# superlinear-ai/raglite

Measured on AMD Instinct MI355X. Metric: queries/sec, MaxSim 32x1M d=1024 exact top-100, higher is better.
Workload: dtype f32 in / f32 scores: candidate chunks found with the fp16 hi halves of corpus and queries (1 x v_mfma_f32_16x16x32_f16 per multiply, f32 accumulate, rigorous error bound), their scores by v_mfma_f32_16x16x4_f32 (exact f32 products); full-precision fallback: 3 x v_mfma_f32_16x16x32_f16 on hi+lo pairs

## Files before the change

include/raglite_hip.h:

```cpp
#ifndef RAGLITE_HIP_H
#define RAGLITE_HIP_H

#include <stddef.h>
#include <stdint.h>

#ifdef __cplusplus
extern "C" {
#endif

typedef enum {
    RL_OK = 0,
    RL_ERR_INVALID = -1,
    RL_ERR_HIP = -2,
    RL_ERR_UNSUPPORTED = -3,
    RL_ERR_NOMEM = -4
} rl_status;

typedef enum { RL_MEM_HOST = 0, RL_MEM_DEVICE = 1 } rl_mem;
#define RL_MEM_FILTERS_DEVICE 2
typedef enum {
    RL_ARITH_AUTO = 0,
    RL_ARITH_FP32_EXACT = 1,
    RL_ARITH_F16_SPLIT = 2,
    RL_ARITH_F16_STORED = 3
} rl_arith;
typedef enum { RL_F32 = 0, RL_F16 = 1 } rl_dtype;
typedef enum { RL_COSINE = 0, RL_DOT = 1, RL_L2 = 2 } rl_metric;
typedef enum { RL_SYNTH_UNIFORM = 0, RL_SYNTH_SMALL_INT = 1 } rl_synth_kind;

typedef struct rl_index rl_index;

int rl_version(void);
const char* rl_last_error(void);
int rl_init(int device);
int rl_device_count(int* count);
int rl_device_info(int device, char* name, int len, int* compute_units, int64_t* total_mem);

int rl_dev_alloc(void** ptr, size_t bytes);
int rl_dev_free(void* ptr);
int rl_memcpy_h2d(void* dst, const void* src, size_t bytes, void* stream);
int rl_memcpy_d2h(void* dst, const void* src, size_t bytes, void* stream);
int rl_memcpy_d2d(void* dst, const void* src, size_t bytes, void* stream);
int rl_stream_sync(void* stream);

int rl_synth_fill(float* dst, int64_t start, int64_t count, uint64_t seed, int kind, void* stream);

int rl_pool_norm(const float* tokens, int64_t n_token_rows, int32_t dim,
                 const int64_t* span_begin, const int64_t* span_end, int64_t n_spans,
                 int32_t normalize, double eps, float* out_f32, uint16_t* out_f16,
                 int mem, void* stream);

int rl_adapter_apply(const float* A, const float* queries, int32_t n_queries, int32_t dim,
                     float* out_f32, uint16_t* out_f16, int mem, void* stream);

int rl_index_create(rl_index** out, const float* embeddings, int64_t n_rows, int32_t dim,
                    const int64_t* chunk_offsets, int64_t n_chunks, int metric, int mem, void* stream);
int rl_index_create_f16(rl_index** out, const uint16_t* embeddings_f16, int64_t n_rows, int32_t dim,
                        const int64_t* chunk_offsets, int64_t n_chunks, int metric, int mem, void* stream);
int rl_index_destroy(rl_index* index);
int rl_index_info(const rl_index* index, int64_t* n_rows, int32_t* dim, int64_t* n_chunks, int* metric);
int rl_index_memory(const rl_index* index, int64_t out[8]);

#define RL_IMAGE_PRESPLIT 1u
#define RL_IMAGE_HI 2u
#define RL_IMAGE_HI_PLANE 4u
int rl_index_prepare(rl_index* index, uint32_t images, uint32_t* built, void* stream);

int rl_index_append(rl_index* index, const float* rows, int64_t n_new_rows, const int64_t* new_chunk_sizes,
                    int64_t n_new_chunks, int mem, void* stream);
int rl_index_delete_chunks(rl_index* index, const int64_t* chunk_ordinals, int64_t n, void* stream);
int rl_index_live(rl_index* index, int64_t* live_rows, int64_t* live_chunks, void* stream);
int rl_index_compact(rl_index* index, int64_t* out_remap, int64_t* new_n_rows, int64_t* new_n_chunks, void* stream);

int rl_index_set_arithmetic(rl_index* index, int mode);
int rl_index_arithmetic(rl_index* index, int* in_effect);

typedef enum {
    RL_OPT_HI_SEARCH = 1, RL_OPT_HI_MAXSIM = 2, RL_OPT_HI_PRODUCTS = 3, RL_OPT_PP_PASS = 4, RL_OPT_FUSED_TOPK = 5, RL_OPT_FUSED_HI = 6,
    RL_OPT_FUSED_PP = 7, RL_OPT_FUSED_TOPK_CAP = 8, RL_OPT_FUSED_TOPK_STRIDE = 9, RL_OPT_GEMM_PASS = 10, RL_OPT_QUERY_PAIRS = 11,
    RL_OPT_PLANES_GEMM = 12, RL_OPT_KEEP_IMAGE = 13, RL_OPT_KEEP_HI = 14, RL_OPT_IMAGE_HEADROOM_MB = 15, RL_OPT_ARITHMETIC = 16,
    RL_OPT_EXACT_KTH_THRESHOLD = 17, RL_OPT_FUSED_TWO_ROUNDS = 18, RL_OPT_KEEP_HI_PLANE = 19, RL_OPT_PAIRS_PACKED = 20,
    RL_OPT_F16_EXACT = 21, RL_OPT_LAZY_IMAGES = 22, RL_OPT_FUSED_PP_SAMPLE = 23,
    RL_OPT_LIST_SELECT = 24, RL_OPT_HI_FEW = 25, RL_OPT_TOPK_BLOCK = 26, RL_OPT_HI_PIVOT = 27, RL_OPT_COUNT_ = 28
} rl_option;
enum { RL_OPT_PP_SCHEDULE = 64, RL_OPT_PP_XCD_PASSES = 65 };
int rl_set_default_option(int key, int64_t value);
int rl_get_default_option(int key, int64_t* value);
int rl_index_set_option(rl_index* index, int key, int64_t value);
int rl_index_get_option(rl_index* index, int key, int64_t* value);

int rl_search_rows(rl_index* index, const float* queries, int32_t n_queries, int32_t k,
                   float* out_scores, int32_t* out_rows, int mem, void* stream);

int rl_rank_cut_begin(rl_index* index, const float* queries, int32_t n_queries, int mem, void* stream);
int rl_rank_cut_level(rl_index* index, int level, int64_t rank_limit, uint32_t* out_hist, int mem, void* stream);
int rl_rank_cut_level_done(rl_index* index, int level, const uint32_t* hist_sum, int mem, void* stream);
int rl_rank_cut_ties(rl_index* index, int64_t rank_limit, uint32_t* out_ties, int mem, void* stream);
int rl_rank_cut_finish(rl_index* index, int64_t rank_limit, const uint32_t* ties_before, const uint32_t* chunk_filter, int32_t k,
                       float* out_scores, int32_t* out_rows, int mem, void* stream);

int rl_search_chunks(rl_index* index, const float* queries, int32_t n_queries, int32_t num_hits,
                     int32_t k, float* out_scores, int32_t* out_chunks, int32_t* out_counts,
                     int mem, void* stream);

int rl_maxsim_topk(rl_index* index, const float* query_vecs, int32_t nq, int32_t k,
                   float* out_scores, int32_t* out_chunks, int mem, void* stream);
int rl_maxsim_scores(rl_index* index, const float* query_vecs, int32_t nq, float* out_scores,
                     int mem, void* stream);
int rl_maxsim_topk_batch(rl_index* index, const float* query_vecs, int32_t n_queries, int32_t nq, int32_t k,
                         float* out_scores, int32_t* out_chunks, int mem, void* stream);
int rl_maxsim_topk_batch_f16(rl_index* index, const uint16_t* query_vecs_f16, int32_t n_queries, int32_t nq, int32_t k,
                             float* out_scores, int32_t* out_chunks, int mem, void* stream);

int rl_maxsim_batch_begin(rl_index* index, const float* query_vecs, int32_t n_queries, int32_t nq, int32_t k, float* out_approx, int mem,
                          void* stream);
int rl_maxsim_batch_finish(rl_index* index, const float* query_vecs, const float* all_approx, int32_t world, int32_t rank, float* out_scores,
                           int32_t* out_chunks, int mem, void* stream);

int rl_maxsim_approx_scores(rl_index* index, const float* query_vecs, int32_t n_queries, int32_t nq, int kernel,
                            float* out_scores, float* out_bound, int mem, void* stream);

int rl_maxsim_rerank(rl_index* index, const float* query_vecs, int32_t n_queries, int32_t nq,
                     const int32_t* candidates, int32_t n_cand, float* out_scores, int mem, void* stream);

int rl_merge_topk(const float* in_scores, const int32_t* in_ids, int32_t n_lists, int32_t n_queries,
                  int32_t k_in, int32_t k, float* out_scores, int32_t* out_ids, int mem, void* stream);

#define RL_COMM_ID_BYTES 128
#define RL_ID_SHARD_MISSING (-2)
typedef struct rl_comm rl_comm;
int rl_comm_unique_id(void* out_id );
int rl_comm_init(rl_comm** out, int rank, int world, const void* unique_id);
int rl_comm_info(const rl_comm* comm, int* rank, int* world);
int rl_comm_destroy(rl_comm* comm);
int rl_allgather_topk(rl_comm* comm, const float* local_scores, const int32_t* local_ids, int32_t n_queries, int32_t k,
                      int32_t id_offset, float* out_scores, int32_t* out_ids, void* stream);
int rl_allgather_merge_topk(rl_comm* comm, const float* local_scores, const int32_t* local_ids, int32_t n_queries,
                            int32_t k_in, int32_t id_offset, int32_t k, float* out_scores, int32_t* out_ids, void* stream);
int rl_allreduce_sum_u32(rl_comm* comm, uint32_t* buf, int64_t count, void* stream);
int rl_allgather_u32(rl_comm* comm, const uint32_t* local, int64_t count, uint32_t* out, void* stream);

int rl_topk(const float* scores, int32_t n_queries, int64_t n, int64_t ld, int32_t k,
            float* out_scores, int32_t* out_ids, int mem, void* stream);

typedef struct rl_keyword_index rl_keyword_index;
int rl_keyword_index_create(rl_keyword_index** out, const int64_t* term_off, int32_t n_terms, const int32_t* post_chunk,
                            const int32_t* post_tf, const int32_t* post_term, int64_t n_postings, const float* idf,
                            const float* nrm, int64_t n_chunks, int mem, void* stream);
int rl_keyword_search(rl_keyword_index* kw, const int64_t* q_off, const int32_t* q_terms, int32_t n_queries, int32_t k,
                      const uint32_t* chunk_filter, float* out_scores, int32_t* out_chunks, int32_t* out_counts, int mem,
                      void* stream);
int rl_keyword_index_info(const rl_keyword_index* kw, int32_t* n_terms, int64_t* n_postings, int64_t* n_chunks);
int rl_keyword_index_destroy(rl_keyword_index* kw);
int rl_keyword_index_read(const rl_keyword_index* kw, int64_t* term_off, int32_t* post_chunk, float* post_impact, int mem,
                          void* stream);

typedef struct rl_keyword_store rl_keyword_store;
int rl_keyword_store_create(rl_keyword_store** out);
int rl_keyword_store_destroy(rl_keyword_store* s);
int rl_keyword_store_info(const rl_keyword_store* s, int64_t* n_chunks, int64_t* n_live, int64_t* n_tokens,
                          int64_t* device_bytes);
int rl_keyword_store_append(rl_keyword_store* s, const int32_t* term_ids, const int64_t* offsets, int64_t n_new_chunks,
                            int mem, void* stream);
int rl_keyword_store_delete(rl_keyword_store* s, const int64_t* chunk_ordinals, int64_t n, void* stream);
int rl_keyword_store_count(rl_keyword_store* s, const int32_t* term_rank, int32_t n_terms, int64_t* out_df,
                           int64_t* out_length, int64_t out_totals[3], int mem, void* stream);
int rl_keyword_store_build(rl_keyword_store* s, const float* idf, const float* nrm, rl_keyword_index** out, int mem,
                           void* stream);

int rl_rrf_fuse(const int32_t* lists, int32_t n_lists, int32_t n_queries, int32_t len, const double* weights, int32_t rrf_k,
                int32_t k, double* out_scores, int32_t* out_ids, int32_t* out_counts, int mem, void* stream);
int rl_hybrid_search(rl_index* index, rl_keyword_index* kw, const float* queries, int32_t n_queries, int32_t num_hits,
                     int32_t n_each, const int64_t* q_off, const int32_t* q_terms, const uint32_t* chunk_filter,
                     int64_t rank_limit, const double* weights, int32_t rrf_k, int32_t k, double* out_scores,
                     int32_t* out_chunks, int32_t* out_counts, int mem, void* stream);

int rl_shard_hybrid_fuse(const int32_t* gathered, int32_t world, int32_t n_queries, int32_t num_hits, int32_t n_each, int32_t n_lists,
                         const double* weights, int32_t rrf_k, int32_t k, double* out_scores, int32_t* out_chunks, int32_t* out_counts,
                         int mem, void* stream);

int rl_search_rows_filtered(rl_index* index, const float* queries, int32_t n_queries, int32_t k,
                            const uint32_t* chunk_filter, float* out_scores, int32_t* out_rows, int mem,
                            void* stream);
int rl_search_chunks_filtered(rl_index* index, const float* queries, int32_t n_queries, int32_t num_hits,
                              int32_t k, const uint32_t* chunk_filter, float* out_scores, int32_t* out_chunks,
                              int32_t* out_counts, int mem, void* stream);
int rl_maxsim_topk_filtered(rl_index* index, const float* query_vecs, int32_t nq, int32_t k,
                            const uint32_t* chunk_filter, float* out_scores, int32_t* out_chunks, int mem,
                            void* stream);

int rl_search_rows_ranked(rl_index* index, const float* queries, int32_t n_queries, int32_t k,
                          const uint32_t* chunk_filter, int64_t rank_limit, float* out_scores, int32_t* out_rows,
                          int mem, void* stream);
int rl_search_chunks_ranked(rl_index* index, const float* queries, int32_t n_queries, int32_t num_hits,
                            int32_t k, const uint32_t* chunk_filter, int64_t rank_limit, float* out_scores,
                            int32_t* out_chunks, int32_t* out_counts, int mem, void* stream);

int rl_search_chunks_per_query(rl_index* index, const float* queries, int32_t n_queries, int32_t num_hits, int32_t k,
                               const uint32_t* chunk_filters, int32_t n_filters, const int32_t* query_filter,
                               const int64_t* rank_limits, float* out_scores, int32_t* out_chunks, int32_t* out_counts,
                               int mem, void* stream);
int rl_keyword_search_per_query(rl_keyword_index* kw, const int64_t* q_off, const int32_t* q_terms, int32_t n_queries,
                                int32_t k, const uint32_t* chunk_filters, int32_t n_filters, const int32_t* query_filter,
                                float* out_scores, int32_t* out_chunks, int32_t* out_counts, int mem, void* stream);
int rl_hybrid_search_per_query(rl_index* index, rl_keyword_index* kw, const float* queries, int32_t n_queries,
                               int32_t num_hits, int32_t n_each, const int64_t* q_off, const int32_t* q_terms,
// ... 62 lines not shown
```

raglite_amd/_abi.py:

```python

from __future__ import annotations

import ctypes as C
import functools
import os
from pathlib import Path

LIB_PATH = Path(os.environ.get("RAGLITE_HIP_LIB") or Path(__file__).resolve().parent / "_lib" / "libraglite_hip.so")

RL_OK, RL_ERR_INVALID, RL_ERR_HIP, RL_ERR_UNSUPPORTED, RL_ERR_NOMEM = 0, -1, -2, -3, -4
MEM_HOST, MEM_DEVICE = 0, 1
MEM_FILTERS_DEVICE = 2
METRICS = {"cosine": 0, "dot": 1, "l2": 2}
SYNTH_KINDS = {"uniform": 0, "small_int": 1}
OPTIONS = {
    "hi_search": 1, "hi_maxsim": 2, "hi_products": 3, "pp_pass": 4, "fused_topk": 5, "fused_hi": 6, "fused_pp": 7, "fused_topk_cap": 8,
    "fused_topk_stride": 9, "gemm_pass": 10, "query_pairs": 11, "planes_gemm": 12, "keep_image": 13, "keep_hi": 14,
    "image_headroom_mb": 15, "arithmetic": 16, "exact_kth_threshold": 17, "fused_two_rounds": 18,
    "keep_hi_plane": 19, "pairs_packed": 20, "f16_exact": 21, "lazy_images": 22, "fused_pp_sample": 23, "list_select": 24, "hi_few": 25, "topk_block": 26, "hi_pivot": 27,
}
SCHEDULE_OPTIONS = {"pp_schedule": 64, "pp_xcd_passes": 65}


def option_key(name: str) -> int:
    return OPTIONS[name] if name in OPTIONS else SCHEDULE_OPTIONS[name]

c_void_p, c_int, c_i32, c_i64, c_u64, c_size_t = C.c_void_p, C.c_int, C.c_int32, C.c_int64, C.c_uint64, C.c_size_t
c_double, c_char_p = C.c_double, C.c_char_p

_SIGNATURES = {
    "rl_version": [],
    "rl_last_error": [],
    "rl_init": [c_int],
    "rl_device_count": [C.POINTER(c_int)],
    "rl_device_info": [c_int, c_char_p, c_int, C.POINTER(c_int), C.POINTER(c_i64)],
    "rl_dev_alloc": [C.POINTER(c_void_p), c_size_t],
    "rl_dev_free": [c_void_p],
    "rl_memcpy_h2d": [c_void_p, c_void_p, c_size_t, c_void_p],
    "rl_memcpy_d2h": [c_void_p, c_void_p, c_size_t, c_void_p],
    "rl_memcpy_d2d": [c_void_p, c_void_p, c_size_t, c_void_p],
    "rl_stream_sync": [c_void_p],
    "rl_synth_fill": [c_void_p, c_i64, c_i64, c_u64, c_int, c_void_p],
    "rl_pool_norm": [c_void_p, c_i64, c_i32, c_void_p, c_void_p, c_i64, c_i32, c_double, c_void_p, c_void_p,
                     c_int, c_void_p],
    "rl_adapter_apply": [c_void_p, c_void_p, c_i32, c_i32, c_void_p, c_void_p, c_int, c_void_p],
    "rl_index_create": [C.POINTER(c_void_p), c_void_p, c_i64, c_i32, c_void_p, c_i64, c_int, c_int, c_void_p],
    "rl_index_destroy": [c_void_p],
    "rl_index_info": [c_void_p, C.POINTER(c_i64), C.POINTER(c_i32), C.POINTER(c_i64), C.POINTER(c_int)],
    "rl_index_memory": [c_void_p, C.POINTER(c_i64)],
    "rl_index_prepare": [c_void_p, C.c_uint32, C.POINTER(C.c_uint32), c_void_p],
    "rl_partition_similarity": [c_void_p, c_i64, c_i32, c_void_p, c_i64, c_void_p, c_void_p, c_int, c_void_p],
    "rl_chunk_best_rows": [c_void_p, c_void_p, c_i32, c_void_p, c_i32, c_void_p, c_int, c_void_p],
    "rl_gather_rows": [c_void_p, c_void_p, c_i64, c_void_p, c_int, c_void_p],
    "rl_index_create_f16": [C.POINTER(c_void_p), c_void_p, c_i64, c_i32, c_void_p, c_i64, c_int, c_int, c_void_p],
    "rl_index_append": [c_void_p, c_void_p, c_i64, c_void_p, c_i64, c_int, c_void_p],
    "rl_index_delete_chunks": [c_void_p, c_void_p, c_i64, c_void_p],
    "rl_index_live": [c_void_p, C.POINTER(c_i64), C.POINTER(c_i64), c_void_p],
    "rl_index_compact": [c_void_p, c_void_p, C.POINTER(c_i64), C.POINTER(c_i64), c_void_p],
    "rl_index_filter_stats": [c_void_p, C.POINTER(c_i64), c_void_p],
    "rl_index_set_arithmetic": [c_void_p, c_int],
    "rl_index_arithmetic": [c_void_p, C.POINTER(c_int)],
    "rl_set_default_option": [c_int, c_i64],
    "rl_get_default_option": [c_int, C.POINTER(c_i64)],
    "rl_index_set_option": [c_void_p, c_int, c_i64],
    "rl_index_get_option": [c_void_p, c_int, C.POINTER(c_i64)],
    "rl_search_rows_filtered": [c_void_p, c_void_p, c_i32, c_i32, c_void_p, c_void_p, c_void_p, c_int, c_void_p],
    "rl_search_chunks_filtered": [c_void_p, c_void_p, c_i32, c_i32, c_i32, c_void_p, c_void_p, c_void_p, c_void_p,
                                  c_int, c_void_p],
    "rl_maxsim_topk_filtered": [c_void_p, c_void_p, c_i32, c_i32, c_void_p, c_void_p, c_void_p, c_int, c_void_p],
    "rl_search_rows_ranked": [c_void_p, c_void_p, c_i32, c_i32, c_void_p, c_i64, c_void_p, c_void_p, c_int, c_void_p],
    "rl_search_chunks_ranked": [c_void_p, c_void_p, c_i32, c_i32, c_i32, c_void_p, c_i64, c_void_p, c_void_p, c_void_p,
                                c_int, c_void_p],
    "rl_search_rows": [c_void_p, c_void_p, c_i32, c_i32, c_void_p, c_void_p, c_int, c_void_p],
    "rl_search_chunks": [c_void_p, c_void_p, c_i32, c_i32, c_i32, c_void_p, c_void_p, c_void_p, c_int, c_void_p],
    "rl_maxsim_topk": [c_void_p, c_void_p, c_i32, c_i32, c_void_p, c_void_p, c_int, c_void_p],
    "rl_maxsim_scores": [c_void_p, c_void_p, c_i32, c_void_p, c_int, c_void_p],
    "rl_maxsim_topk_batch": [c_void_p, c_void_p, c_i32, c_i32, c_i32, c_void_p, c_void_p, c_int, c_void_p],
    "rl_maxsim_topk_batch_f16": [c_void_p, c_void_p, c_i32, c_i32, c_i32, c_void_p, c_void_p, c_int, c_void_p],
    "rl_maxsim_approx_scores": [c_void_p, c_void_p, c_i32, c_i32, c_int, c_void_p, c_void_p, c_int, c_void_p],
    "rl_maxsim_batch_begin": [c_void_p, c_void_p, c_i32, c_i32, c_i32, c_void_p, c_int, c_void_p],
    "rl_maxsim_batch_finish": [c_void_p, c_void_p, c_void_p, c_i32, c_i32, c_void_p, c_void_p, c_int, c_void_p],
    "rl_maxsim_rerank": [c_void_p, c_void_p, c_i32, c_i32, c_void_p, c_i32, c_void_p, c_int, c_void_p],
    "rl_merge_topk": [c_void_p, c_void_p, c_i32, c_i32, c_i32, c_i32, c_void_p, c_void_p, c_int, c_void_p],
    "rl_topk": [c_void_p, c_i32, c_i64, c_i64, c_i32, c_void_p, c_void_p, c_int, c_void_p],
    "rl_time_kernel": [c_void_p, c_int, c_void_p, c_i32, c_i32, C.POINTER(C.c_float), c_void_p],
    "rl_comm_unique_id": [c_void_p],
    "rl_comm_init": [C.POINTER(c_void_p), c_int, c_int, c_void_p],
    "rl_comm_info": [c_void_p, C.POINTER(c_int), C.POINTER(c_int)],
    "rl_comm_destroy": [c_void_p],
    "rl_allgather_topk": [c_void_p, c_void_p, c_void_p, c_i32, c_i32, c_i32, c_void_p, c_void_p, c_void_p],
    "rl_allgather_merge_topk": [c_void_p, c_void_p, c_void_p, c_i32, c_i32, c_i32, c_i32, c_void_p, c_void_p, c_void_p],
    "rl_allreduce_sum_u32": [c_void_p, c_void_p, c_i64, c_void_p],
    "rl_allgather_u32": [c_void_p, c_void_p, c_i64, c_void_p, c_void_p],
    "rl_rank_cut_begin": [c_void_p, c_void_p, c_i32, c_int, c_void_p],
    "rl_rank_cut_level": [c_void_p, c_int, c_i64, c_void_p, c_int, c_void_p],
    "rl_rank_cut_level_done": [c_void_p, c_int, c_void_p, c_int, c_void_p],
    "rl_rank_cut_ties": [c_void_p, c_i64, c_void_p, c_int, c_void_p],
    "rl_rank_cut_finish": [c_void_p, c_i64, c_void_p, c_void_p, c_i32, c_void_p, c_void_p, c_int, c_void_p],
    "rl_keyword_index_create": [C.POINTER(c_void_p), c_void_p, c_i32, c_void_p, c_void_p, c_void_p, c_i64, c_void_p, c_void_p, c_i64,
                                c_int, c_void_p],
    "rl_keyword_search": [c_void_p, c_void_p, c_void_p, c_i32, c_i32, c_void_p, c_void_p, c_void_p, c_void_p, c_int, c_void_p],
    "rl_keyword_index_info": [c_void_p, C.POINTER(c_i32), C.POINTER(c_i64), C.POINTER(c_i64)],
    "rl_keyword_index_destroy": [c_void_p],
    "rl_keyword_index_read": [c_void_p, c_void_p, c_void_p, c_void_p, c_int, c_void_p],
    "rl_keyword_store_create": [C.POINTER(c_void_p)],
    "rl_keyword_store_destroy": [c_void_p],
    "rl_keyword_store_info": [c_void_p, C.POINTER(c_i64), C.POINTER(c_i64), C.POINTER(c_i64), C.POINTER(c_i64)],
    "rl_keyword_store_append": [c_void_p, c_void_p, c_void_p, c_i64, c_int, c_void_p],
    "rl_keyword_store_delete": [c_void_p, c_void_p, c_i64, c_void_p],
    "rl_keyword_store_count": [c_void_p, c_void_p, c_i32, c_void_p, c_void_p, c_void_p, c_int, c_void_p],
    "rl_keyword_store_build": [c_void_p, c_void_p, c_void_p, C.POINTER(c_void_p), c_int, c_void_p],
    "rl_rrf_fuse": [c_void_p, c_i32, c_i32, c_i32, c_void_p, c_i32, c_i32, c_void_p, c_void_p, c_void_p, c_int, c_void_p],
    "rl_shard_hybrid_fuse": [c_void_p, c_i32, c_i32, c_i32, c_i32, c_i32, c_void_p, c_i32, c_i32, c_void_p, c_void_p, c_void_p, c_int,
                             c_void_p],
    "rl_hybrid_search": [c_void_p, c_void_p, c_void_p, c_i32, c_i32, c_i32, c_void_p, c_void_p, c_void_p, c_i64, c_void_p, c_i32, c_i32,
                         c_void_p, c_void_p, c_void_p, c_int, c_void_p],
    "rl_search_chunks_per_query": [c_void_p, c_void_p, c_i32, c_i32, c_i32, c_void_p, c_i32, c_void_p, c_void_p, c_void_p, c_void_p,
                                   c_void_p, c_int, c_void_p],
    "rl_keyword_search_per_query": [c_void_p, c_void_p, c_void_p, c_i32, c_i32, c_void_p, c_i32, c_void_p, c_void_p, c_void_p, c_void_p,
                                    c_int, c_void_p],
    "rl_hybrid_search_per_query": [c_void_p, c_void_p, c_void_p, c_i32, c_i32, c_i32, c_void_p, c_void_p, c_void_p, c_i32, c_void_p,
                                   c_void_p, c_void_p, c_i32, c_i32, c_void_p, c_void_p, c_void_p, c_int, c_void_p],
    "rl_rerank_order": [c_void_p, c_void_p, c_i32, c_i32, c_i32, c_void_p, c_void_p, c_void_p, c_void_p, c_int, c_void_p],
    "rl_search_rerank_per_query": [c_void_p, c_void_p, c_void_p, c_i32, c_i32, c_i32, c_void_p, c_void_p, c_void_p, c_i32, c_void_p,
                                   c_void_p, c_void_p, c_i32, c_i32, c_void_p, c_i32, c_i32, c_void_p, c_void_p, c_void_p, c_int,
                                   c_void_p],
    "rl_span_table_create": [C.POINTER(c_void_p), c_void_p, c_void_p, c_i64],
    "rl_span_table_info": [c_void_p, C.POINTER(c_i64), C.POINTER(c_i64), C.POINTER(c_i64)],
    "rl_span_table_destroy": [c_void_p],
    "rl_chunk_spans": [c_void_p, c_void_p, c_i32, c_i32, c_void_p, c_i32, c_void_p, c_void_p, c_void_p, c_void_p, c_void_p, c_int, c_void_p],
    "rl_search_rerank_spans_per_query": [c_void_p, c_void_p, c_void_p, c_i32, c_i32, c_i32, c_void_p, c_void_p, c_void_p, c_i32, c_void_p,
                                         c_void_p, c_void_p, c_i32, c_i32, c_void_p, c_i32, c_i32, c_void_p, c_void_p, c_i32, c_void_p,
                                         c_void_p, c_void_p, c_void_p, c_void_p, c_void_p, c_void_p, c_int, c_void_p],
    "rl_metadata_store_create": [C.POINTER(c_void_p), c_void_p, c_void_p, c_i64, c_int, c_void_p],
    "rl_metadata_store_append": [c_void_p, c_void_p, c_void_p, c_i64, c_int, c_void_p],
    "rl_metadata_store_memory": [c_void_p, C.POINTER(c_i64)],
    "rl_metadata_store_destroy": [c_void_p],
    "rl_metadata_filters": [c_void_p, c_void_p, c_void_p, c_void_p, c_i32, C.POINTER(c_void_p), c_void_p, c_void_p, c_int, c_void_p],
    "rl_filter_set_bits": [c_void_p, C.POINTER(c_void_p), C.POINTER(c_i32), C.POINTER(c_i64)],
    "rl_filter_set_read": [c_void_p, c_void_p, c_int, c_void_p],
    "rl_filter_set_destroy": [c_void_p],
}
COMM_ID_BYTES = 128
_RESTYPES = {"rl_last_error": c_char_p}
EXPORTED_SYMBOLS = tuple(_SIGNATURES)


class RagliteHipError(RuntimeError):
    """HIP runtime failure inside libraglite_hip.so."""


class UnsupportedError(ValueError):
    """RL_ERR_UNSUPPORTED: the arguments are valid but this entry point does not cover them (a ValueError, as before; its own type so
    that callers with another path -- `ShardedIndex.maxsim_topk_batch` -- can take it)."""


@functools.lru_cache(maxsize=1)
def lib() -> C.CDLL:
    if not LIB_PATH.exists():
        raise ImportError(
            f"{LIB_PATH} not found: build it with `python -m raglite_amd._build` (needs hipcc; "
            "cross-compiles for gfx950 without a GPU). raglite_amd has no CPU fallback."
        )
    try:
        import torch
# ... 48 lines not shown
```

raglite_amd/_ops.py:

```python

from __future__ import annotations

import ctypes as C
import threading
from typing import Any

import numpy as np

from raglite_amd import _abi
from raglite_amd._abi import MEM_DEVICE, MEM_FILTERS_DEVICE, MEM_HOST, METRICS, SYNTH_KINDS, check, lib

K_MAX = 2048


def _is_torch(x: Any) -> bool:
    return type(x).__module__.split(".")[0] == "torch"


def _torch():
    import torch

    return torch


# ... 861 lines not shown
    def maxsim_topk(self, query_vecs, k: int, chunk_filter=None):
        a = _Args()
        p_q, nq, _ = self._queries(a, query_vecs)
        o_s, p_s = a.out((k,), np.float32)
        o_c, p_c = a.out((k,), np.int32)
        p_f = self._filter(a, chunk_filter)
        self._prep(a)
        check(lib().rl_maxsim_topk_filtered(self._handle, p_q, nq, k, p_f, p_s, p_c, a.mem, a.stream))
        return o_s, o_c

    def maxsim_topk_batch(self, query_batch, k: int):
        a = _Args()
        half = _is_half(query_batch)
        p_q = a.inp(query_batch, np.float16 if half else np.float32)
        qv = a.keep[-1]
        if qv.ndim != 3 or int(qv.shape[2]) != self.dim:
            raise ValueError("query_batch must be (n_queries, nq, dim)")
        n_queries, nq = int(qv.shape[0]), int(qv.shape[1])
        o_s, p_s = a.out((n_queries, k), np.float32)
        o_c, p_c = a.out((n_queries, k), np.int32)
        self._prep(a)
        fn = lib().rl_maxsim_topk_batch_f16 if half else lib().rl_maxsim_topk_batch
        check(fn(self._handle, p_q, n_queries, nq, k, p_s, p_c, a.mem, a.stream))
        return o_s, o_c

    def maxsim_approx_scores(self, query_batch, kernel: int = 0):
        a = _Args()
        p_q = a.inp(query_batch, np.float32)
        qv = a.keep[-1]
        if qv.ndim != 3 or int(qv.shape[2]) != self.dim:
            raise ValueError("query_batch must be (n_queries, nq, dim)")
        n_queries, nq = int(qv.shape[0]), int(qv.shape[1])
        o_s, p_s = a.out((n_queries, self.n_chunks), np.float32)
        o_b, p_b = a.out((n_queries,), np.float32)
        self._prep(a)
        check(lib().rl_maxsim_approx_scores(self._handle, p_q, n_queries, nq, int(kernel), p_s, p_b, a.mem, a.stream))
        return o_s, o_b

    def maxsim_batch_begin(self, query_batch, k: int):
        a = _Args()
        p_q = a.inp(query_batch, np.float32)
        qv = a.keep[-1]
        if qv.ndim != 3 or int(qv.shape[2]) != self.dim:
            raise ValueError("query_batch must be (n_queries, nq, dim)")
        n_queries, nq = int(qv.shape[0]), int(qv.shape[1])
        o, p_o = a.out((n_queries, int(k) + 1), np.float32)
        self._prep(a)
        check(lib().rl_maxsim_batch_begin(self._handle, p_q, n_queries, nq, int(k), p_o, a.mem, a.stream))
        return o

    def maxsim_batch_finish(self, query_batch, all_approx, rank: int, k: int):
        a = _Args()
        p_q = a.inp(query_batch, np.float32)
        qv = a.keep[-1]
        n_queries = int(qv.shape[0])
        p_a = a.inp(all_approx, np.float32)
        av = a.keep[-1]
        if av.ndim != 3 or int(av.shape[1]) != n_queries or int(av.shape[2]) != int(k) + 1:
            raise ValueError("all_approx must be (world, n_queries, k + 1)")
        world = int(av.shape[0])
        o_s, p_s = a.out((n_queries, int(k)), np.float32)
        o_c, p_c = a.out((n_queries, int(k)), np.int32)
        self._prep(a)
        check(lib().rl_maxsim_batch_finish(self._handle, p_q, p_a, world, int(rank), p_s, p_c, a.mem, a.stream))
        return o_s, o_c

    def maxsim_rerank(self, query_vecs, candidates):
        a = _Args()
        p_q = a.inp(query_vecs, np.float32)
        qv = a.keep[-1]
        if qv.ndim != 3 or int(qv.shape[2]) != self.dim:
            raise ValueError("query_vecs must be (n_queries, nq, dim)")
        p_c = a.inp(candidates, np.int32)
        cv = a.keep[-1]
        n_queries, nq = int(qv.shape[0]), int(qv.shape[1])
        if cv.ndim != 2 or int(cv.shape[0]) != n_queries:
            raise ValueError("candidates must be (n_queries, n_cand)")
        n_cand = int(cv.shape[1])
        o_s, p_s = a.out((n_queries, n_cand), np.float32)
        self._prep(a)
        check(lib().rl_maxsim_rerank(self._handle, p_q, n_queries, nq, p_c, n_cand, p_s, a.mem, a.stream))
        return o_s

    def chunk_best_rows(self, queries, candidates):
        a = _Args()
        p_q, B, single = self._queries(a, queries)
        c2 = candidates.reshape(1, -1) if candidates.ndim == 1 else candidates
        p_c = a.inp(c2, np.int32)
        if int(a.keep[-1].shape[0]) != B:
            raise ValueError("candidates must have one row per query")
        n_cand = int(a.keep[-1].shape[1])
        o_r, p_r = a.out((B, n_cand), np.int32)
        self._prep(a)
        check(lib().rl_chunk_best_rows(self._handle, p_q, B, p_c, n_cand, p_r, a.mem, a.stream))
        return o_r[0] if single else o_r

    def gather_rows(self, rows):
        a = _Args()
        p_r = a.inp(rows, np.int32)
        n = int(a.keep[0].shape[0])
        o, p_o = a.out((n, self.dim), np.float32)
        self._prep(a)
        check(lib().rl_gather_rows(self._handle, p_r, n, p_o, a.mem, a.stream))
        return o

    def time_kernel(self, kind: int, query_vecs_cuda, iters: int) -> float:
        a = _Args()
        p_q, nq, _ = self._queries(a, query_vecs_cuda)
        if a.mem != MEM_DEVICE:
            raise ValueError("time_kernel needs CUDA tensors")
        ms = C.c_float(0.0)
        self._prep(a)
        check(lib().rl_time_kernel(self._handle, kind, p_q, nq, iters, C.byref(ms), a.stream))
        return float(ms.value)


class KeywordIndex:

    def __init__(self, postings) -> None:
        p = postings
        arrs = [np.ascontiguousarray(p.term_off, dtype=np.int64), np.ascontiguousarray(p.post_chunk, dtype=np.int32),
                np.ascontiguousarray(p.post_tf, dtype=np.int32), np.ascontiguousarray(p.post_term, dtype=np.int32),
                np.ascontiguousarray(p.idf, dtype=np.float32), np.ascontiguousarray(p.nrm, dtype=np.float32)]
        term_off, post_chunk, post_tf, post_term, idf, nrm = arrs
        self.n_terms, self.n_postings, self.n_chunks = int(term_off.size - 1), int(post_chunk.size), int(nrm.size)
        _ensure_init(_current_device())
        handle = C.c_void_p()
        check(lib().rl_keyword_index_create(C.byref(handle), term_off.ctypes.data, self.n_terms, post_chunk.ctypes.data,
                                            post_tf.ctypes.data, post_term.ctypes.data, self.n_postings, idf.ctypes.data,
                                            nrm.ctypes.data, self.n_chunks, MEM_HOST, None))
        self._handle = handle

    @classmethod
    def _from_handle(cls, handle) -> "KeywordIndex":
        self = cls.__new__(cls)
        n_terms, n_postings, n_chunks = C.c_int32(0), C.c_int64(0), C.c_int64(0)
        self._handle = handle
        check(lib().rl_keyword_index_info(handle, C.byref(n_terms), C.byref(n_postings), C.byref(n_chunks)))
        self.n_terms, self.n_postings, self.n_chunks = n_terms.value, n_postings.value, n_chunks.value
        return self

    def read(self):
        term_off = np.empty(self.n_terms + 1, np.int64)
        post_chunk = np.empty(self.n_postings, np.int32)
        post_impact = np.empty(self.n_postings, np.float32)
        _ensure_init(_current_device())
        check(lib().rl_keyword_index_read(self._handle, term_off.ctypes.data, post_chunk.ctypes.data, post_impact.ctypes.data, MEM_HOST, None))
        return term_off, post_chunk, post_impact

    def close(self) -> None:
        h, self._handle = getattr(self, "_handle", None), None
        if h:
            lib().rl_keyword_index_destroy(h)

    def __del__(self) -> None:
        try:
            self.close()
        except Exception:
            pass

    def search(self, query_term_ids, k: int, chunk_filter=None, *, query_filters=None):
        q_off, q_terms = _term_csr(query_term_ids)
        B = int(q_off.size - 1)
        scores = np.empty((B, k), np.float32)
        chunks = np.empty((B, k), np.int32)
        counts = np.empty(B, np.int32)
# ... 96 lines not shown
```

raglite_amd/csrc/api.hip:

```cpp
#include <cmath>
#include <cstdlib>
#include <cstring>
#include <limits>
#include <memory>
#include <mutex>
#include <utility>
#include <vector>

#include "common.h"

namespace rl {

static thread_local std::string g_last_error;
void set_error(const std::string& msg) { g_last_error = msg; }
int fail(int code, const std::string& msg) {
    g_last_error = msg;
    return code;
}

namespace {

hipStream_t as_stream(void* s) { return reinterpret_cast<hipStream_t>(s); }

struct BlockCache {
// ... 100 lines not shown
        if (bytes <= cap) return RL_OK;
        release();
        RL_HIP(hipMalloc(&p, bytes));
        cap = bytes;
        return RL_OK;
    }
    int alloc(size_t bytes, const char* who) {
        release();
        RL_TRY(hip_status(hipMalloc(&p, bytes), who));
        cap = bytes;
        return RL_OK;
    }
    void release() {
        if (p) (void)hipFree(p);
        p = nullptr;
        cap = 0;
    }
    template <class T>
    T* as() const { return reinterpret_cast<T*>(p); }
};
template <class T>
struct DevArray : Pool {
    operator T*() const { return as<T>(); }
};

template <class T>
int stage_in(const T* src, size_t count, int mem, hipStream_t s, DevBuf& tmp, const T** out) {
    if (mem == RL_MEM_DEVICE) { *out = src; return RL_OK; }
    RL_TRY(tmp.alloc(count * sizeof(T)));
    if (count) {
        const void* from = src;
        if (void* pin = g_pinned.take(count * sizeof(T))) {
            std::memcpy(pin, src, count * sizeof(T));
            from = pin;
        }
        RL_HIP(hipMemcpyAsync(tmp.p, from, count * sizeof(T), hipMemcpyHostToDevice, s));
    }
    *out = tmp.as<T>();
    return RL_OK;
}
template <class T>
int stage_out_begin(T* dst, size_t count, int mem, DevBuf& tmp, T** out) {
    if (mem == RL_MEM_DEVICE || dst == nullptr) { *out = dst; return RL_OK; }
    RL_TRY(tmp.alloc(count * sizeof(T)));
    *out = tmp.as<T>();
    return RL_OK;
}
template <class T>
int stage_out_end(T* dst, size_t count, int mem, hipStream_t s, const DevBuf& tmp) {
    if (mem == RL_MEM_DEVICE || dst == nullptr || count == 0) return RL_OK;
    if (void* pin = g_pinned.take(count * sizeof(T))) {
        RL_HIP(hipMemcpyAsync(pin, tmp.p, count * sizeof(T), hipMemcpyDeviceToHost, s));
        g_pinned.pending.push_back({&tmp, pin, dst, count * sizeof(T)});
        return RL_OK;
    }
    RL_HIP(hipMemcpyAsync(dst, tmp.p, count * sizeof(T), hipMemcpyDeviceToHost, s));
    return RL_OK;
}
int sync_and_drain(hipStream_t s) {
    RL_HIP(hipStreamSynchronize(s));
    g_pinned.drain();
    return RL_OK;
}
int finish(int mem, hipStream_t s) {
    if (mem == RL_MEM_HOST) return sync_and_drain(s);
    return RL_OK;
}

int filters_mem(int mem) { return (mem & RL_MEM_FILTERS_DEVICE) ? RL_MEM_DEVICE : mem; }
int args_mem(int mem) { return mem & ~RL_MEM_FILTERS_DEVICE; }

int scan_mode(int metric) {
    switch (metric) {
        case RL_COSINE: return SCAN_COSINE;
        case RL_DOT: return SCAN_DOT;
        case RL_L2: return SCAN_L2;
        default: return -1;
    }
}

constexpr size_t SCORE_BATCH_BYTES = size_t(8) << 30;

struct Options {
    int64_t v[RL_OPT_PP_XCD_PASSES + 1];
    Options() {
        for (auto& x : v) x = 0;
        v[RL_OPT_HI_SEARCH] = v[RL_OPT_HI_MAXSIM] = v[RL_OPT_HI_PRODUCTS] = v[RL_OPT_PP_PASS] = v[RL_OPT_FUSED_TOPK] = v[RL_OPT_FUSED_HI] = 1;
        v[RL_OPT_FUSED_PP] = v[RL_OPT_GEMM_PASS] = v[RL_OPT_QUERY_PAIRS] = v[RL_OPT_PLANES_GEMM] = v[RL_OPT_KEEP_IMAGE] = v[RL_OPT_KEEP_HI] = 1;
        v[RL_OPT_EXACT_KTH_THRESHOLD] = v[RL_OPT_FUSED_TWO_ROUNDS] = v[RL_OPT_KEEP_HI_PLANE] = v[RL_OPT_F16_EXACT] = v[RL_OPT_LAZY_IMAGES] = v[RL_OPT_FUSED_PP_SAMPLE] = v[RL_OPT_LIST_SELECT] = v[RL_OPT_HI_FEW] = 1;
        v[RL_OPT_TOPK_BLOCK] = v[RL_OPT_PAIRS_PACKED] = 2;
        v[RL_OPT_HI_PIVOT] = 1;
        v[RL_OPT_PP_SCHEDULE] = 1;
        v[RL_OPT_PP_XCD_PASSES] = 2;
        v[RL_OPT_IMAGE_HEADROOM_MB] = -1;
        v[RL_OPT_ARITHMETIC] = RL_ARITH_AUTO;
    }
    bool on(int key) const { return v[key] != 0; }
};
std::mutex g_default_opts_mu;
Options g_default_opts;
bool option_key_ok(int key) { return (key >= 1 && key < RL_OPT_COUNT_) || key == RL_OPT_PP_SCHEDULE || key == RL_OPT_PP_XCD_PASSES; }
bool option_value_ok(int key, int64_t value) {
    switch (key) {
        case RL_OPT_HI_SEARCH: case RL_OPT_HI_MAXSIM: case RL_OPT_PP_PASS: case RL_OPT_FUSED_TOPK: case RL_OPT_FUSED_HI: case RL_OPT_FUSED_PP:
        case RL_OPT_GEMM_PASS: case RL_OPT_QUERY_PAIRS: case RL_OPT_PLANES_GEMM: case RL_OPT_KEEP_IMAGE: case RL_OPT_KEEP_HI:
        case RL_OPT_EXACT_KTH_THRESHOLD: case RL_OPT_FUSED_TWO_ROUNDS: case RL_OPT_KEEP_HI_PLANE: case RL_OPT_F16_EXACT: case RL_OPT_LAZY_IMAGES: case RL_OPT_FUSED_PP_SAMPLE: case RL_OPT_LIST_SELECT: case RL_OPT_HI_FEW: case RL_OPT_HI_PIVOT:
        case RL_OPT_PP_SCHEDULE:
            return value == 0 || value == 1;
        case RL_OPT_PP_XCD_PASSES: return value == 8 || value == 4 || value == 2 || value == 1;
        case RL_OPT_TOPK_BLOCK: case RL_OPT_PAIRS_PACKED: return value >= 0 && value <= 2;
        case RL_OPT_HI_PRODUCTS: return value == 1 || value == 2;
        case RL_OPT_FUSED_TOPK_CAP: return value >= 0 && value <= MERGE_CAP;
        case RL_OPT_FUSED_TOPK_STRIDE: return value == 0 || (value >= 2 && value <= (int64_t(1) << 20));
        case RL_OPT_IMAGE_HEADROOM_MB: return value >= -1 && value <= (int64_t(1) << 30);
        case RL_OPT_ARITHMETIC: return value == RL_ARITH_AUTO || value == RL_ARITH_FP32_EXACT;
        default: return false;
    }
}

struct Image {
    Pool buf;
    float scale = 0.f;
    int64_t rows = 0;
    void drop() {
        buf.release();
        scale = 0.f;
        rows = 0;
    }
    bool covers(float at, int64_t n_rows) const { return scale > 0.f && scale == at && rows == n_rows && n_rows > 0; }
};
struct NormStats {
    float max_row_norm = 0.f, max_lo_norm = 0.f, max_lo_ratio = 0.f;
    float min_row_norm = std::numeric_limits<float>::infinity();
    float max_row_norm_scale = 0.f;
    int64_t max_row_norm_rows = 0;
    void reset() { *this = NormStats(); }
    bool measured(int64_t n_rows) const { return max_row_norm_rows == n_rows && max_row_norm > 0.f; }
};

}
}

struct rl_index {
    const float* E = nullptr;
    const uint16_t* E16 = nullptr;
    rl::Pool owned_rows;
    bool owns_E() const { return owned_rows.p != nullptr; }
    int64_t n_rows = 0;
    int32_t dim = 0;
    int64_t n_chunks = 0;
    int metric = RL_COSINE;
    bool has_empty_chunk = false;
    rl::DevArray<int64_t> offsets;
    rl::DevArray<int32_t> row_to_chunk;
    rl::DevArray<float> norm;
    rl::DevArray<float> sumsq;
    int n_cu = 256;
    std::mutex mu;
    rl::SelectWorkspace ws;
    rl::Pool scores;
    rl::Pool hits;
    rl::Pool misc;
    int64_t cap_rows = 0;
    int64_t cap_chunks = 0;
    std::vector<int64_t> h_offsets;
    std::vector<uint32_t> h_live;
    rl::DevArray<uint32_t> live_chunk_bits;
    rl::DevArray<uint32_t> live_row_bits;
    int64_t n_dead_chunks = 0, n_dead_rows = 0;
    rl::Pool maskbuf;
    rl::Pool qsplit;
    rl::DevArray<uint32_t> d_range;
    float max_abs = 0.f, min_row_max = std::numeric_limits<float>::infinity();
    bool nonfinite = false;
    int arithmetic = RL_ARITH_AUTO;
    float split_scale = 0.f;
    rl::Image planes;
    rl::Pool ends, qplanes;
    rl::Pool q32;
    rl::Pool cand;
    rl::Pool fused;
    rl::Pool pp_work;
    rl::Pool rankbuf;
    rl::Pool hybrid;
    rl::Pool rerank;
    rl::Image hiplane;
    rl::Pool hibuf;
    rl::Image hi_image;
    rl::NormStats norm_stats;
    rl::DevArray<uint32_t> d_norms;
// ... 1651 lines not shown
    }
    RL_TRY(maxsim_scores_device(idx, d_q, nq, idx->scores.as<float>(), s));
    const bool masked = d_f || idx->live_chunk_bits;
    RL_TRY(mask_chunk_scores(idx, idx->scores.as<float>(), 1, idx->n_chunks, d_f, s));
    RL_TRY(launch_topk(idx->scores.as<float>(), 1, idx->n_chunks, idx->n_chunks, k, idx->ws, d_s, d_c, s));
    if (masked) RL_TRY(launch_fix_masked(d_s, d_c, k, s));
    RL_TRY(stage_out_end(out_scores, (size_t)k, mem, s, t_s));
    RL_TRY(stage_out_end(out_chunks, (size_t)k, mem, s, t_c));
    return finish(mem, s);
}

int rl_maxsim_topk(rl_index* idx, const float* query_vecs, int32_t nq, int32_t k, float* out_scores,
                   int32_t* out_chunks, int mem, void* stream) {
    return rl_maxsim_topk_filtered(idx, query_vecs, nq, k, nullptr, out_scores, out_chunks, mem, stream);
}

namespace {
struct HiBatch {
    float* ts; int32_t* ti; float* thr; uint32_t* cnt; uint32_t* flag; int32_t* ci; float* es;
    float* m; float* es_top;
    int32_t cap; bool one_product; float m_abs; const float* q_unscale;
    uint64_t* bmax = nullptr;
    const float* qsum = nullptr;
    bool m_ready = true;
    bool exact_kth;
    const uint32_t* filter = nullptr;
};
void hi_batch_layout(rl_index* idx, int32_t n, int32_t k, HiBatch& hb) {
    hb.cap = 2048;
    hb.ts = idx->hibuf.as<float>();
    hb.ti = reinterpret_cast<int32_t*>(hb.ts + (size_t)n * k);
    hb.thr = reinterpret_cast<float*>(hb.ti + (size_t)n * k);
    hb.cnt = reinterpret_cast<uint32_t*>(hb.thr + n);
    hb.flag = hb.cnt + n;
    hb.ci = reinterpret_cast<int32_t*>(hb.flag + 16);
    hb.es = reinterpret_cast<float*>(hb.ci + (size_t)n * hb.cap);
    hb.m = hb.es + (size_t)n * hb.cap;
    hb.es_top = hb.m + n;
    hb.bmax = reinterpret_cast<uint64_t*>((reinterpret_cast<uintptr_t>(hb.es_top + (size_t)n * k) + 7) & ~uintptr_t(7));
}
size_t hi_batch_words(int32_t n, int32_t k) {
    return (size_t)n * k * 3 + (size_t)n * 3 + 16 + (size_t)n * 2048 * 2 + 2 + 2 * pivot_scratch_words(std::min<int32_t>(n, 2));
}
int hi_batch_approx(rl_index* idx, const float* d_q, int32_t nq, int32_t n_queries, int32_t n_gemm, int32_t k, float* sc, int64_t ld, HiBatch& hb,
                    hipStream_t s, bool flag_zeroed = false) {
    hb.one_product = idx->opt.v[RL_OPT_HI_PRODUCTS] == 1;
    hb.exact_kth = idx->opt.on(RL_OPT_EXACT_KTH_THRESHOLD);
    RL_TRY(idx->hibuf.reserve(hi_batch_words(n_gemm, k) * 4));
    hi_batch_layout(idx, n_gemm, k, hb);
    const int32_t cap = hb.cap;
    hb.m_abs = idx->norm_stats.max_lo_norm + sum_eps(idx->dim) * idx->norm_stats.max_row_norm;
    hb.q_unscale = reinterpret_cast<const float*>(idx->qplanes.as<char>() + (size_t)n_queries * idx->dim * 128);
    hb.qsum = hb.q_unscale + 2 * (size_t)n_queries;
    if (!flag_zeroed) RL_HIP(hipMemsetAsync(hb.flag, 0, 16 * sizeof(uint32_t), s));
    (void)cap;
    const bool pp = hb.one_product && idx->dim >= 256 && idx->opt.on(RL_OPT_PP_PASS);
    if (pp)
        RL_TRY(launch_maxsim_pp(approx_image(idx), idx->n_rows, idx->dim, idx->qplanes.p, n_queries, 0, n_gemm, nq, idx->row_to_chunk,
                                idx->offsets, idx->ends.as<uint32_t>(), sc, ld, idx->n_cu, s, approx_scale(idx), nullptr,
                                (int)idx->opt.v[RL_OPT_PP_SCHEDULE], (int)idx->opt.v[RL_OPT_PP_XCD_PASSES]));
    for (int32_t b = 0; !pp && b < n_gemm; b += GEMM_PASS_QUERIES) {
        const int32_t n_q = std::min<int32_t>(GEMM_PASS_QUERIES, n_gemm - b);
        RL_TRY(launch_maxsim_gemm(approx_image(idx), idx->n_rows, idx->dim, idx->qplanes.p, n_queries, b, n_q, nq, idx->row_to_chunk,
                                  idx->offsets, idx->ends.as<uint32_t>(), sc + (int64_t)b * ld, ld, idx->n_cu, s, approx_scale(idx), true,
                                  nullptr, hb.one_product));
    }
    RL_TRY(mask_chunk_scores(idx, sc, n_gemm, ld, hb.filter, s));
    int st_pv = RL_ERR_UNSUPPORTED;
    if (n_gemm < 16 && idx->n_chunks > (int64_t)262144 && idx->opt.on(RL_OPT_HI_PIVOT))
        st_pv = launch_topk_pivot(sc, n_gemm, idx->n_chunks, ld, k, idx->ws, hb.ts, hb.ti, s);
    if (st_pv != RL_OK && st_pv != RL_ERR_UNSUPPORTED) return st_pv;
    if (st_pv == RL_ERR_UNSUPPORTED) RL_TRY(launch_topk(sc, n_gemm, idx->n_chunks, ld, k, idx->ws, hb.ts, hb.ti, s));
    return RL_OK;
}
int hi_batch_fallback(rl_index* idx, const float* d_q, int32_t nq, int32_t n_queries, int32_t n_gemm, int32_t k, float* sc, int64_t ld,
                      const HiBatch& hb, float* d_s, int32_t* d_c, hipStream_t s, bool rows_only = false);
int hi_batch_rescore(rl_index* idx, const float* d_q, int32_t nq, int32_t n_queries, int32_t n_gemm, int32_t k, float* sc, int64_t ld,
                     const HiBatch& hb, float* d_s, int32_t* d_c, hipStream_t s, bool rows_only = false) {
    const size_t q_elems = (size_t)nq * idx->dim;
    const float* rows = idx->E16 ? reinterpret_cast<const float*>(idx->E16) : idx->E;
    const bool rows16 = idx->E16 != nullptr;
    idx->filt = {RL_FILTER_MAXSIM_BATCH, n_gemm, hb.cap, hb.cnt, hb.flag};
    const int packed = (int)idx->opt.v[RL_OPT_PAIRS_PACKED];
    const bool m_from_qsum = !hb.m_ready && hb.qsum != nullptr;
    if (!hb.m_ready && !(hb.exact_kth && k <= hb.cap && hb.qsum)) return fail(RL_ERR_INVALID, "MaxSim batch: no bound for the candidate threshold");
    if (hb.exact_kth && k <= hb.cap) {
        RL_TRY(launch_maxsim_pairs(rows, idx->dim, d_q, nq, (int64_t)q_elems, idx->offsets, hb.ti, k, n_gemm, hb.es_top, s, rows16, 0, 0, packed));
        if (m_from_qsum)
            RL_TRY(launch_exact_threshold(hb.es_top, hb.ti, n_gemm, k, hb.m, hb.cap, hb.thr, hb.cnt, hb.ci, hb.es, hb.flag, s, hb.qsum, hb.m_abs,
                                          idx->norm_stats.max_row_norm + idx->norm_stats.max_lo_norm, hb.one_product, hb.ts));
        else
            RL_TRY(launch_exact_threshold(hb.es_top, hb.ti, n_gemm, k, hb.m, hb.cap, hb.thr, hb.cnt, hb.ci, hb.es, hb.flag, s, nullptr, 0.f, 0.f, false, hb.ts));
        RL_TRY(launch_collect_above(sc, n_gemm, idx->n_chunks, ld, hb.thr, nullptr, hb.cap, hb.ci, nullptr, hb.cnt, hb.flag, s, hb.ts, hb.ti, k));
        if (hb.cap > k)
            RL_TRY(launch_maxsim_pairs(rows, idx->dim, d_q, nq, (int64_t)q_elems, idx->offsets, hb.ci, hb.cap - k, n_gemm, hb.es, s, rows16, hb.cap, k, packed));
    } else {
        RL_HIP(hipMemsetAsync(hb.ci, 0xff, (size_t)n_gemm * hb.cap * sizeof(int32_t), s));
        RL_TRY(launch_collect_above(sc, n_gemm, idx->n_chunks, ld, hb.thr, nullptr, hb.cap, hb.ci, nullptr, hb.cnt, hb.flag, s));
        RL_TRY(launch_maxsim_pairs(rows, idx->dim, d_q, nq, (int64_t)q_elems, idx->offsets, hb.ci, hb.cap, n_gemm, hb.es, s, rows16, 0, 0, packed));
    }
    RL_TRY(launch_merge_topk(hb.es, hb.ci, 1, n_gemm, hb.cap, k, d_s, d_c, s, hb.cnt));
    return hi_batch_fallback(idx, d_q, nq, n_queries, n_gemm, k, sc, ld, hb, d_s, d_c, s, rows_only);
}
int hi_batch_fallback(rl_index* idx, const float* d_q, int32_t nq, int32_t n_queries, int32_t n_gemm, int32_t k, float* sc, int64_t ld,
                      const HiBatch& hb, float* d_s, int32_t* d_c, hipStream_t s, bool rows_only) {
    const size_t q_elems = (size_t)nq * idx->dim;
    if (image_valid(idx) && !rows_only)
        RL_TRY(launch_maxsim_gemm(idx->planes.buf.p, idx->n_rows, idx->dim, idx->qplanes.p, n_queries, 0, n_gemm, nq, idx->row_to_chunk, idx->offsets,
                                  idx->ends.as<uint32_t>(), sc, ld, idx->n_cu, s, image_scale(idx), idx->E16 != nullptr, hb.flag, false, true));
    else if (idx->dim > 1024)
        RL_TRY(launch_maxsim_pairs_all_wide(idx->E, idx->dim, d_q, nq, (int64_t)q_elems, idx->offsets, idx->n_chunks, n_gemm, sc, ld, s, hb.flag));
    else
        RL_TRY(launch_maxsim_stream_batch(idx->E, false, idx->n_rows, idx->dim, d_q, nq, (int64_t)q_elems, n_gemm, idx->row_to_chunk, idx->offsets,
                                          idx->n_chunks, sc, ld, std::max(1, idx->n_cu / std::min<int32_t>(8, std::max<int32_t>(1, n_gemm / 4))), s,
                                          idx->split_scale, hb.flag));
    RL_TRY(mask_chunk_scores(idx, sc, n_gemm, ld, hb.filter, s));
    uint32_t* host_word = nullptr;
    if (idx->opt.on(RL_OPT_LAZY_IMAGES) && !image_valid(idx) && !rows_only) {
        if (!idx->h_fell_back) {
            void* word = nullptr;
            if (hipHostMalloc(&word, sizeof(uint32_t), hipHostMallocMapped) == hipSuccess) {
                idx->h_fell_back.reset(static_cast<uint32_t*>(word));
                *idx->h_fell_back = 0u;
                if (hipHostGetDevicePointer(reinterpret_cast<void**>(&idx->d_fell_back), word, 0) != hipSuccess) {
                    idx->d_fell_back = nullptr;
                    (void)hipGetLastError();
                }
            } else (void)hipGetLastError();
        }
        if (idx->h_fell_back) host_word = idx->d_fell_back;
        if (idx->h_fell_back && !host_word) {
            RL_TRY(launch_guarded_select(sc, n_gemm, idx->n_chunks, ld, k, nullptr, nullptr, nullptr, 0, SCAN_RAW_DOT, 1.0f, d_s, d_c, hb.flag, s));
            RL_HIP(hipMemcpyAsync(idx->h_fell_back.get(), hb.flag, sizeof(uint32_t), hipMemcpyDeviceToHost, s));
            return RL_OK;
        }
    }
    RL_TRY(launch_guarded_select(sc, n_gemm, idx->n_chunks, ld, k, nullptr, nullptr, nullptr, 0, SCAN_RAW_DOT, 1.0f, d_s, d_c, hb.flag, s, host_word));
    return RL_OK;
}

int maxsim_few_hi_plane(rl_index* idx, const float* d_q, int32_t nq, int32_t n, int32_t k, float* sc, int64_t ld, float* d_s, int32_t* d_c,
                        hipStream_t s, const uint32_t* d_filter) {
    if (n < 1 || n > 2 || nq < 1 || nq > 32 || k > 512 || !idx->opt.on(RL_OPT_HI_MAXSIM) || !idx->opt.on(RL_OPT_HI_FEW)) return RL_ERR_UNSUPPORTED;
    if (idx->dim > 1024) return RL_ERR_UNSUPPORTED;
    if (idx->E16 || !idx->E || !(idx->split_scale > 0.f) || idx->has_empty_chunk || idx->n_chunks == 0 || idx->n_rows == 0) return RL_ERR_UNSUPPORTED;
    RL_TRY(demand_images(idx, IMG_HI_PLANE, s));
    if (!hi_valid(idx) || !idx->norm_stats.measured(idx->n_rows)) return RL_ERR_UNSUPPORTED;
    if ((reinterpret_cast<uintptr_t>(d_q) & 15) || (reinterpret_cast<uintptr_t>(idx->E) & 15)) return RL_ERR_UNSUPPORTED;
    const int64_t q_elems = (int64_t)nq * idx->dim;
    int st = RL_ERR_UNSUPPORTED;
    if (n == 2 && nq > 16 && idx->opt.on(RL_OPT_QUERY_PAIRS)) {
        RL_TRY(idx->qsplit.reserve(query_split_bytes(idx->dim, 2)));
        st = launch_query_split(d_q, idx->dim, nq, q_elems, 2, idx->qsplit.as<char>(), true, s);
        if (st == RL_OK)
            st = launch_maxsim_stream2(idx->hiplane.buf.p, true, idx->n_rows, idx->dim, idx->qsplit.as<char>(), 2, 0, nq, idx->row_to_chunk, idx->offsets,
                                       idx->n_chunks, sc, ld, idx->n_cu, s, 1.f);
    }
    if (st == RL_ERR_UNSUPPORTED)
        st = launch_maxsim_stream_batch(idx->hiplane.buf.p, true, idx->n_rows, idx->dim, d_q, nq, q_elems, n, idx->row_to_chunk, idx->offsets,
                                        idx->n_chunks, sc, ld, idx->n_cu, s, 0.f, nullptr);
    if (st != RL_OK) return st;
    HiBatch hb;
    hb.one_product = false;
    hb.exact_kth = idx->opt.on(RL_OPT_EXACT_KTH_THRESHOLD);
    RL_TRY(idx->hibuf.reserve(hi_batch_words(n, k) * 4));
    hi_batch_layout(idx, n, k, hb);
    hb.m_abs = idx->norm_stats.max_lo_norm + sum_eps(idx->dim) * idx->norm_stats.max_row_norm;
    hb.q_unscale = nullptr;
    hb.filter = d_filter;
    if (idx->opt.on(RL_OPT_HI_PIVOT) && !idx->live_chunk_bits && !d_filter && k <= 128) {
        HiBound bound;
        bound.m_out = hb.m;
        PivotMaxSim ms;
        ms.nq = nq; ms.q_stride = q_elems; ms.m_abs = hb.m_abs; ms.fill_ids = hb.ci;
        const int st_pv = launch_pivot_route(sc, n, idx->n_chunks, ld, k, nullptr, nullptr, d_q, idx->dim, SCAN_RAW_DOT, 1.0f / idx->split_scale, hb.bmax,
                                             hb.cnt, n + 16, bound, hb.thr, hb.cap, hb.ci, nullptr, hb.cnt, hb.flag, s, nullptr, nullptr, nullptr, &ms);
        if (st_pv == RL_OK) {
            idx->filt = {RL_FILTER_MAXSIM_BATCH, n, hb.cap, hb.cnt, hb.flag};
            RL_TRY(launch_maxsim_pairs(idx->E, idx->dim, d_q, nq, q_elems, idx->offsets, hb.ci, hb.cap, n, hb.es, s, false, 0, 0,
                                       std::min<int>(1, (int)idx->opt.v[RL_OPT_PAIRS_PACKED])));
            RL_TRY(launch_merge_topk(hb.es, hb.ci, 1, n, hb.cap, k, d_s, d_c, s, hb.cnt));
            return hi_batch_fallback(idx, d_q, nq, n, n, k, sc, ld, hb, d_s, d_c, s, true);
// ... 235 lines not shown
    RL_TRY(stage_out_begin(out_scores, (size_t)n_queries * ld, mem, t_o, &d_o));
    if (out_bound) RL_TRY(stage_out_begin(out_bound, (size_t)n_queries, mem, t_b, &d_b));
    RL_TRY(idx->qplanes.reserve(query_planes_bytes(idx->dim, n_queries)));
    RL_TRY(launch_query_planes(d_q, idx->dim, nq, (int64_t)q_elems, n_queries, idx->qplanes.p, s));
    const int32_t per = kernel == 0 ? n_queries : GEMM_PASS_QUERIES;
    for (int32_t b = 0; b < n_queries; b += per) {
        const int32_t n_q = std::min<int32_t>(per, n_queries - b);
        if (kernel == 0)
            RL_TRY(launch_maxsim_pp(approx_image(idx), idx->n_rows, idx->dim, idx->qplanes.p, n_queries, b, n_q, nq, idx->row_to_chunk, idx->offsets,
                                    idx->ends.as<uint32_t>(), d_o + (int64_t)b * ld, ld, idx->n_cu, s, approx_scale(idx), nullptr,
                                    (int)idx->opt.v[RL_OPT_PP_SCHEDULE], (int)idx->opt.v[RL_OPT_PP_XCD_PASSES]));
        else
            RL_TRY(launch_maxsim_gemm(approx_image(idx), idx->n_rows, idx->dim, idx->qplanes.p, n_queries, b, n_q, nq, idx->row_to_chunk, idx->offsets,
                                      idx->ends.as<uint32_t>(), d_o + (int64_t)b * ld, ld, idx->n_cu, s, approx_scale(idx), true, nullptr, true));
    }
    if (d_b) {
        const float m_abs = idx->norm_stats.max_lo_norm + sum_eps(idx->dim) * idx->norm_stats.max_row_norm;
        const float* q_unscale = reinterpret_cast<const float*>(idx->qplanes.as<char>() + (size_t)n_queries * idx->dim * 128);
        RL_TRY(idx->hibuf.reserve((size_t)n_queries * 4 * sizeof(float) + 64));
        float* top = idx->hibuf.as<float>();
        float* thr = top + n_queries;
        uint32_t* cnt = reinterpret_cast<uint32_t*>(thr + n_queries);
        uint32_t* flag = cnt + n_queries;
        RL_HIP(hipMemsetAsync(top, 0, (size_t)n_queries * sizeof(float), s));
        RL_HIP(hipMemsetAsync(flag, 0, 16 * sizeof(uint32_t), s));
        RL_TRY(launch_maxsim_threshold(top, n_queries, 1, d_q, nq, idx->dim, (int64_t)q_elems, 1.0f, m_abs, thr, cnt, flag, s, q_unscale,
                                       idx->norm_stats.max_row_norm + idx->norm_stats.max_lo_norm));
        RL_TRY(launch_scale_f32(thr, d_b, -0.5f, n_queries, s));
        idx->filt = {};
    }
    RL_TRY(stage_out_end(out_scores, (size_t)n_queries * ld, mem, s, t_o));
    if (out_bound) RL_TRY(stage_out_end(out_bound, (size_t)n_queries, mem, s, t_b));
    return finish(mem, s);
}

}

namespace {
int maxsim_rerank_device(rl_index* idx, const float* d_q, int32_t n_queries, int32_t nq, const int32_t* d_c, int32_t n_cand, float* d_o,
                         hipStream_t s) {
    {
        const int64_t n_items = (int64_t)n_queries * n_cand;
        RL_TRY(idx->cand.reserve((size_t)n_items * sizeof(int32_t)));
        RL_TRY(launch_sanitize_candidates(d_c, n_items, idx->n_chunks, idx->live_chunk_bits, idx->cand.as<int32_t>(), s));
        d_c = idx->cand.as<int32_t>();
    }
    int st = idx->E16 ? launch_maxsim_cand16(idx->E16, idx->dim, d_q, nq, idx->offsets, d_c, n_cand, n_queries, d_o, s)
                      : launch_maxsim_cand(idx->E, idx->dim, d_q, nq, idx->offsets, d_c, n_cand, n_queries, d_o, s, idx->split_scale);
    if (st == RL_ERR_UNSUPPORTED)
        st = launch_maxsim_pairs(idx->E16 ? reinterpret_cast<const float*>(idx->E16) : idx->E, idx->dim, d_q, nq, (int64_t)nq * idx->dim, idx->offsets, d_c,
                                 n_cand, n_queries, d_o, s, idx->E16 != nullptr, 0, 0, (int)idx->opt.v[RL_OPT_PAIRS_PACKED]);
    if (st == RL_ERR_UNSUPPORTED && idx->E16) return fail(st, "rl_maxsim_rerank: unsupported shape for an fp16-stored index");
    if (st == RL_ERR_UNSUPPORTED && !idx->E16)
        st = launch_maxsim_generic(idx->E, idx->dim, d_q, nq, (int64_t)nq * idx->dim, idx->offsets, d_c, n_cand,
                                   n_queries, d_o, s);
    return st;
}
}

extern "C" {

int rl_maxsim_rerank(rl_index* idx, const float* query_vecs, int32_t n_queries, int32_t nq, const int32_t* candidates,
                     int32_t n_cand, float* out_scores, int mem, void* stream) {
    if (!idx) return fail(RL_ERR_INVALID, "rl_maxsim_rerank: null index");
    if (n_queries < 0 || n_cand < 0 || nq < 1) return fail(RL_ERR_INVALID, "rl_maxsim_rerank: bad sizes");
    if (n_queries == 0 || n_cand == 0) return RL_OK;
    if (!query_vecs || !candidates || !out_scores) return fail(RL_ERR_INVALID, "rl_maxsim_rerank: null argument");
    if (idx->E16 && (nq > 32 || idx->dim % 16))
        return fail(RL_ERR_UNSUPPORTED, "rl_maxsim_rerank on an fp16-stored index needs nq <= 32 and dim % 16 == 0");
    if (mem == RL_MEM_HOST) {
        for (int64_t i = 0; i < (int64_t)n_queries * n_cand; ++i)
            if (candidates[i] < -1 || candidates[i] >= idx->n_chunks)
                return fail(RL_ERR_INVALID, "rl_maxsim_rerank: candidate chunk ordinal out of range");
    }
    hipStream_t s = as_stream(stream);
    std::lock_guard<std::mutex> lock(idx->mu);
    RL_TRY(use_scratch(idx, s));
    DevBuf t_q, t_c, t_o;
    const float* d_q; const int32_t* d_c; float* d_o;
    RL_TRY(stage_in(query_vecs, (size_t)n_queries * nq * idx->dim, mem, s, t_q, &d_q));
    RL_TRY(stage_in(candidates, (size_t)n_queries * n_cand, mem, s, t_c, &d_c));
    RL_TRY(stage_out_begin(out_scores, (size_t)n_queries * n_cand, mem, t_o, &d_o));
    RL_TRY(maxsim_rerank_device(idx, d_q, n_queries, nq, d_c, n_cand, d_o, s));
    RL_TRY(stage_out_end(out_scores, (size_t)n_queries * n_cand, mem, s, t_o));
    return finish(mem, s);
}

int rl_merge_topk(const float* in_scores, const int32_t* in_ids, int32_t n_lists, int32_t n_queries, int32_t k_in,
                  int32_t k, float* out_scores, int32_t* out_ids, int mem, void* stream) {
    if (n_lists < 1 || n_queries < 0 || k_in < 1 || k < 1) return fail(RL_ERR_INVALID, "rl_merge_topk: bad sizes");
    if (k > K_MAX) return fail(RL_ERR_UNSUPPORTED, "rl_merge_topk: k must be <= 2048");
    if (n_queries == 0) return RL_OK;
    if (!in_scores || !in_ids || !out_scores || !out_ids) return fail(RL_ERR_INVALID, "rl_merge_topk: null argument");
    hipStream_t s = as_stream(stream);
    const size_t n_in = (size_t)n_lists * n_queries * k_in, n_out = (size_t)n_queries * k;
    DevBuf t_is, t_ii, t_os, t_oi;
    const float* d_is; const int32_t* d_ii; float* d_os; int32_t* d_oi;
    RL_TRY(stage_in(in_scores, n_in, mem, s, t_is, &d_is));
    RL_TRY(stage_in(in_ids, n_in, mem, s, t_ii, &d_ii));
    RL_TRY(stage_out_begin(out_scores, n_out, mem, t_os, &d_os));
    RL_TRY(stage_out_begin(out_ids, n_out, mem, t_oi, &d_oi));
    RL_TRY(launch_merge_topk(d_is, d_ii, n_lists, n_queries, k_in, k, d_os, d_oi, s));
    RL_TRY(stage_out_end(out_scores, n_out, mem, s, t_os));
    RL_TRY(stage_out_end(out_ids, n_out, mem, s, t_oi));
    return finish(mem, s);
}

int rl_topk(const float* scores, int32_t n_queries, int64_t n, int64_t ld, int32_t k, float* out_scores,
            int32_t* out_ids, int mem, void* stream) {
    if (n_queries < 0 || n < 0 || ld < n || k < 1) return fail(RL_ERR_INVALID, "rl_topk: bad sizes");
    if (k > K_MAX) return fail(RL_ERR_UNSUPPORTED, "rl_topk: k must be <= 2048");
    if (n_queries == 0) return RL_OK;
    if ((n > 0 && !scores) || !out_scores || !out_ids) return fail(RL_ERR_INVALID, "rl_topk: null argument");
    hipStream_t s = as_stream(stream);
    const size_t n_in = (size_t)n_queries * ld, n_out = (size_t)n_queries * k;
    DevBuf t_in, t_os, t_oi;
    const float* d_in; float* d_os; int32_t* d_oi;
    RL_TRY(stage_in(scores, n_in, mem, s, t_in, &d_in));
    RL_TRY(stage_out_begin(out_scores, n_out, mem, t_os, &d_os));
    RL_TRY(stage_out_begin(out_ids, n_out, mem, t_oi, &d_oi));
    SelectWorkspace ws;
    {
        std::lock_guard<std::mutex> lock(g_default_opts_mu);
        ws.block_route = (int)g_default_opts.v[RL_OPT_TOPK_BLOCK];
    }
    int st = launch_topk(d_in, n_queries, n, ld, k, ws, d_os, d_oi, s);
    if (st == RL_OK) st = stage_out_end(out_scores, n_out, mem, s, t_os);
    if (st == RL_OK) st = stage_out_end(out_ids, n_out, mem, s, t_oi);
    const int sy = sync_and_drain(s);
    select_workspace_free(ws);
    return st == RL_OK ? sy : st;
}

int rl_partition_similarity(const float* X, int64_t n, int32_t dim, const int64_t* doc_offsets, int64_t n_docs,
                            const uint8_t* nonoutlying, float* out, int mem, void* stream) {
    if (n < 0 || dim <= 0) return fail(RL_ERR_INVALID, "rl_partition_similarity: bad shape");
    if (n == 0) return RL_OK;
    if (!X || !out) return fail(RL_ERR_INVALID, "rl_partition_similarity: null argument");
    if (dim > 4096) return fail(RL_ERR_UNSUPPORTED, "rl_partition_similarity: dim must be <= 4096");
    if (!doc_offsets) n_docs = 1;
    if (n_docs < 1) return fail(RL_ERR_INVALID, "rl_partition_similarity: need at least one document");
    hipStream_t s = as_stream(stream);
    DevBuf t_x, t_off, t_sel, t_out, t_scr, t_one;
    const float* d_x; const int64_t* d_off; const uint8_t* d_sel = nullptr; float* d_out;
    RL_TRY(stage_in(X, (size_t)n * dim, mem, s, t_x, &d_x));
    if (doc_offsets) {
        RL_TRY(stage_in(doc_offsets, (size_t)n_docs + 1, mem, s, t_off, &d_off));
    } else {
        const int64_t one[2] = {0, n};
        RL_TRY(t_one.alloc(sizeof(one)));
        RL_HIP(hipMemcpyAsync(t_one.p, one, sizeof(one), hipMemcpyHostToDevice, s));
        RL_HIP(hipStreamSynchronize(s));
        d_off = t_one.as<int64_t>();
    }
    if (nonoutlying) RL_TRY(stage_in(nonoutlying, (size_t)n, mem, s, t_sel, &d_sel));
    RL_TRY(stage_out_begin(out, (size_t)n, mem, t_out, &d_out));
    RL_TRY(t_scr.alloc(partition_sim_scratch_bytes(n, n_docs, dim)));
    RL_TRY(launch_partition_similarity(d_x, n, dim, d_off, n_docs, d_sel, d_out, t_scr.p, s));
    RL_TRY(stage_out_end(out, (size_t)n, mem, s, t_out));
    return sync_and_drain(s);
}

int rl_chunk_best_rows(rl_index* idx, const float* queries, int32_t B, const int32_t* candidates, int32_t n_cand,
                       int32_t* out_rows, int mem, void* stream) {
    if (!idx) return fail(RL_ERR_INVALID, "rl_chunk_best_rows: null index");
    if (B < 0 || n_cand < 0) return fail(RL_ERR_INVALID, "rl_chunk_best_rows: bad sizes");
// ... 1293 lines not shown
```

raglite_amd/csrc/common.h:

```cpp
#pragma once
#include <hip/hip_runtime.h>
#include <stdint.h>

#include <algorithm>
#include <cstdlib>
#include <string>

#include "raglite_hip.h"

namespace rl {

void set_error(const std::string& msg);
int fail(int code, const std::string& msg);

#define RL_HIP(expr)                                                                         \
    do {                                                                                     \
        hipError_t _e = (expr);                                                              \
        if (_e != hipSuccess)                                                                \
            return ::rl::fail(_e == hipErrorOutOfMemory ? RL_ERR_NOMEM : RL_ERR_HIP,         \
                              std::string(#expr) + ": " + hipGetErrorString(_e));            \
    } while (0)

#define RL_TRY(expr)              \
    do {                          \
// ... 305 lines not shown
int launch_permute_rows(const int32_t* rows_in, const int32_t* pos, int32_t k, int64_t n_items, int32_t* rows_out,
                        hipStream_t s);
int launch_gather_rows(const void* E, bool f16, int32_t dim, int64_t n_rows, const int32_t* rows, int64_t n, float* out,
                       hipStream_t s, const uint32_t* counts = nullptr, int32_t cap = 0);
int launch_compact_rows(const void* src, int64_t row_bytes, const int64_t* old_row, int64_t n, void* dst, hipStream_t s);

size_t partition_sim_scratch_bytes(int64_t n, int64_t n_docs, int32_t dim);
int launch_partition_similarity(const float* X, int64_t n, int32_t dim, const int64_t* doc_off, int64_t n_docs,
                                const uint8_t* sel, float* out, void* scratch, hipStream_t s);

int launch_row_to_chunk(const int64_t* chunk_offsets, int64_t n_chunks, int64_t n_rows, int32_t* row_to_chunk,
                        hipStream_t s);
int launch_maxsim_stream(const float* D, int64_t n_rows, int32_t dim, const float* Q, int32_t nq,
                         const int32_t* row_to_chunk, const int64_t* chunk_offsets, int64_t n_chunks, int mode,
                         float* out, int64_t ld, int n_cu, hipStream_t s, float split_scale = 0.f,
                         const uint32_t* run_if = nullptr);
struct StreamSecondJob {
    const float* D = nullptr;
    int64_t n_rows = 0;
    float* out = nullptr;
    int64_t ld = 0;
    const uint32_t* run_if = nullptr;
};
int launch_maxsim_stream_two(const float* D, int64_t n_rows, int32_t dim, const float* Q, int32_t nq, const int32_t* row_to_chunk,
                             const int64_t* chunk_offsets, int64_t n_chunks, float* out, int64_t ld, int n_cu, hipStream_t s, float split_scale,
                             const StreamSecondJob& job2);
int launch_maxsim_stream_batch(const void* D, bool f16, int64_t n_rows, int32_t dim, const float* Q, int32_t nq, int64_t q_stride,
                               int32_t n_queries, const int32_t* row_to_chunk, const int64_t* chunk_offsets, int64_t n_chunks, float* out,
                               int64_t out_stride, int n_cu, hipStream_t s, float split_scale, const uint32_t* run_if = nullptr);
size_t query_split_bytes(int32_t dim, int32_t n_queries);
int launch_query_split(const float* Q, int32_t dim, int32_t nq, int64_t q_stride, int32_t n_queries, void* buf, bool f16_corpus,
                       hipStream_t s);
int launch_maxsim_stream2(const void* D, bool f16, int64_t n_rows, int32_t dim, const void* split_buf, int32_t n_queries,
                          int32_t first, int32_t nq, const int32_t* row_to_chunk, const int64_t* chunk_offsets, int64_t n_chunks,
                          float* out, int64_t out_stride, int n_cu, hipStream_t s, float split_scale);
size_t planes_bytes(int64_t rows, int32_t dim, bool half = false);
int launch_presplit_rows(const float* E, int64_t first_row, int64_t n_rows, int32_t dim, float scale, void* planes, hipStream_t s);
int launch_preformat_rows16(const uint16_t* E, int64_t first_row, int64_t n_rows, int32_t dim, void* planes, hipStream_t s);
int launch_presplit_hi_rows(const float* E, int64_t first_row, int64_t n_rows, int32_t dim, float scale, void* planes, hipStream_t s);
size_t chunk_ends_words(int64_t rows);
int launch_chunk_ends(const int32_t* row_to_chunk, int64_t n_rows, uint32_t* ends, hipStream_t s);
size_t query_planes_bytes(int32_t dim, int32_t n_queries);
int launch_query_planes(const float* Q, int32_t dim, int32_t nq, int64_t q_stride, int32_t n_queries, void* buf, hipStream_t s,
                        uint32_t* zero_words = nullptr, int n_zero = 0);
int launch_maxsim_gemm(const void* planes, int64_t n_rows, int32_t dim, const void* qbuf, int32_t n_queries, int32_t first,
                       int32_t n_q, int32_t nq, const int32_t* row_to_chunk, const int64_t* chunk_offsets, const uint32_t* ends_bits,
                       float* out, int64_t out_stride, int n_cu, hipStream_t s, float split_scale, bool half = false,
                       const uint32_t* run_if = nullptr, bool hi_only = false, bool all_passes = false);
constexpr int32_t PP_PASS_QUERIES = 16;
int launch_maxsim_pp(const void* image, int64_t n_rows, int32_t dim, const void* qbuf, int32_t n_queries, int32_t first, int32_t n_q,
                     int32_t nq, const int32_t* row_to_chunk, const int64_t* chunk_offsets, const uint32_t* ends_bits, float* out,
                     int64_t out_stride, int n_cu, hipStream_t s, float split_scale, const uint32_t* run_if, int schedule, int xcd_passes);
constexpr int32_t MFMA_RATE_ITERS = 1000;
int launch_mfma_f16_rate(float* out, int n_cu, int32_t iters, hipStream_t s, double* flops);
size_t score_planes_scratch_floats(int32_t nb, int32_t dim);
int launch_score_planes(const void* planes, int64_t n_rows, int32_t dim, const float* Q, int32_t nb, float* scores, int64_t ld,
                        const float* row_norm, const float* row_sumsq, float* scratch, int mode, int n_cu, hipStream_t s, float split_scale,
                        bool half = false);
struct CandArgs { const float* tau; int32_t tau_stride; float* scores; int32_t* ids; uint32_t* cnt; uint32_t* overflow; int32_t cap; };
int launch_score_planes_queries(const float* Q, int32_t nb, int32_t dim, float* scratch, int mode, hipStream_t s, uint32_t* zero_word = nullptr);
size_t pp_rows_scratch_bytes(int64_t n_rows, int32_t nb, int n_cu, int32_t expected_per_query, int32_t* log_cap_out);
int launch_pp_rows_pass(const void* image, int64_t n_rows, int32_t dim, int32_t nb, float* scratch, const float* row_norm, int mode,
                        const CandArgs* cand, void* work, int32_t log_cap, int n_cu, hipStream_t s, float split_scale, int64_t tile_begin = 0,
                        int64_t tile_count = -1, bool norms_ready = false,
                        bool row_norm_test = false);
int launch_pp_rows_sample(const void* image, int64_t n_rows, int32_t dim, int32_t nb, float* scratch, const float* row_norm, int mode, float* S,
                          int64_t ld_s, int32_t stride, int n_cu, hipStream_t s, float split_scale);
int launch_raise_threshold(float* thr, const float* kth, int32_t nq, int32_t k, const float* window, hipStream_t s);
int launch_score_planes_pass(const void* planes, int64_t n_rows, int32_t dim, int32_t nb, float* scratch, float* scores, int64_t ld,
                             const float* row_norm, const float* row_sumsq, int mode, int32_t tile_stride, const uint32_t* run_if,
                             const CandArgs* cand, int n_cu, hipStream_t s, float split_scale, bool half = false, bool hi_only = false);
int launch_row_range(const float* E, int64_t n_rows, int32_t dim, uint32_t* range, hipStream_t s);
int launch_score_gemm(const float* E, int64_t n_rows, int32_t dim, const float* Q, int32_t nb, float* scores,
                      int64_t ld, const float* row_norm, const float* row_sumsq, float* q_sumsq_scratch, int mode,
                      int n_cu, hipStream_t s, float split_scale = 0.f);
size_t score_gemm_scratch_floats(int32_t nb, int32_t dim, bool split);
int launch_maxsim_stream16(const uint16_t* D, int64_t n_rows, int32_t dim, const float* Q, int32_t nq,
                           const int32_t* row_to_chunk, const int64_t* chunk_offsets, int64_t n_chunks, int mode,
                           float* out, int64_t ld, int n_cu, hipStream_t s);
int launch_maxsim_pairs(const float* D, int32_t dim, const float* Q, int32_t nq, int64_t q_stride, const int64_t* chunk_offsets,
                        const int32_t* candidates, int64_t n_items_per_query, int32_t n_queries, float* out, hipStream_t s,
                        bool rows16 = false,
                        int64_t item_stride = 0, int64_t first_item = 0,
                        int packed = 1);
int launch_maxsim_pairs_all_wide(const float* D, int32_t dim, const float* Q, int32_t nq, int64_t q_stride, const int64_t* offsets, int64_t n_chunks,
                                 int32_t n_queries, float* out, int64_t out_stride, hipStream_t s, const uint32_t* run_if, bool rows16 = false);
int launch_maxsim_generic(const float* D, int32_t dim, const float* Q, int32_t nq, int64_t q_stride_queries,
                          const int64_t* chunk_offsets, const int32_t* candidates, int64_t n_items,
                          int32_t n_queries, float* out, hipStream_t s);
int launch_sanitize_candidates(const int32_t* in, int64_t n, int64_t n_chunks, const uint32_t* live_chunk_bits, int32_t* out,
                               hipStream_t s);
int launch_maxsim_cand(const float* D, int32_t dim, const float* Q, int32_t nq, const int64_t* chunk_offsets,
                       const int32_t* candidates, int32_t n_cand, int32_t n_queries, float* out, hipStream_t s,
                       float split_scale = 0.f);
int launch_maxsim_cand16(const uint16_t* D, int32_t dim, const float* Q, int32_t nq, const int64_t* chunk_offsets,
                         const int32_t* candidates, int32_t n_cand, int32_t n_queries, float* out, hipStream_t s);

}
```

raglite_amd/csrc/maxsim_generic.hip:

```cpp
#include "common.h"

namespace rl {

typedef float f32x4 __attribute__((ext_vector_type(4)));
typedef _Float16 h16x8 __attribute__((ext_vector_type(8)));

constexpr int GEN_NQ_MAX = 1024;
constexpr int PAIRS_MAX_DIM = 4096;

template <int NV, int VEC>
__global__ __launch_bounds__(256) void maxsim_generic_kernel(const float* __restrict__ D, int dim,
                                                              const float* __restrict__ Q, int nq,
                                                              const int64_t* __restrict__ offsets,
                                                              const int32_t* __restrict__ candidates,
                                                              int64_t n_items, float* __restrict__ out) {
    __shared__ float msh[4][GEN_NQ_MAX];
    const int lane = threadIdx.x & 63;
    const int w = threadIdx.x >> 6;
    float* m = msh[w];
    const int64_t wave0 = (int64_t)blockIdx.x * 4 + w;
    const int64_t n_waves = (int64_t)gridDim.x * 4;
    for (int64_t item = wave0; item < n_items; item += n_waves) {
        const int64_t chunk = candidates ? (int64_t)candidates[item] : item;
        const int64_t b = chunk >= 0 ? offsets[chunk] : 0, e = chunk >= 0 ? offsets[chunk + 1] : 0;
        for (int i = lane; i < nq; i += 64) m[i] = -INFINITY;
        for (int64_t r = b; r < e; ++r) {
            float x[NV][VEC];
#pragma unroll
            for (int v = 0; v < NV; ++v) {
                const int c = (v * 64 + lane) * VEC;
#pragma unroll
                for (int j = 0; j < VEC; ++j) x[v][j] = 0.f;
                if (c < dim) {
                    if constexpr (VEC == 4) {
                        const float4 t = *reinterpret_cast<const float4*>(D + r * (int64_t)dim + c);
                        x[v][0] = t.x; x[v][1] = t.y; x[v][2] = t.z; x[v][3] = t.w;
                    } else {
                        x[v][0] = D[r * (int64_t)dim + c];
                    }
                }
            }
            for (int i = 0; i < nq; ++i) {
                float s = 0.f;
#pragma unroll
                for (int v = 0; v < NV; ++v) {
                    const int c = (v * 64 + lane) * VEC;
                    if (c < dim) {
                        if constexpr (VEC == 4) {
                            const float4 t = *reinterpret_cast<const float4*>(Q + (int64_t)i * dim + c);
                            s = fmaf(x[v][0], t.x, s); s = fmaf(x[v][1], t.y, s);
                            s = fmaf(x[v][2], t.z, s); s = fmaf(x[v][3], t.w, s);
                        } else {
                            s = fmaf(x[v][0], Q[(int64_t)i * dim + c], s);
                        }
                    }
                }
                s = wave_sum(s);
                if (lane == 0) m[i] = fmaxf(m[i], s);
            }
        }
        float t = 0.f;
        for (int i = lane; i < nq; i += 64) t += m[i];
        t = wave_sum(t);
        if (lane == 0) out[item] = (e > b) ? t : -INFINITY;
    }
}

template <int NV, int VEC>
static int generic_t(const float* D, int32_t dim, const float* Q, int32_t nq, const int64_t* offsets,
                     const int32_t* cand, int64_t n_items, float* out, hipStream_t s) {
    const int blocks = (int)std::max<int64_t>(1, std::min<int64_t>((n_items + 3) / 4, 256 * 8));
    hipLaunchKernelGGL((maxsim_generic_kernel<NV, VEC>), dim3(blocks), dim3(256), 0, s, D, (int)dim, Q, (int)nq,
                       offsets, cand, n_items, out);
    RL_HIP(hipGetLastError());
    return RL_OK;
}

template <bool FULL, int KB, bool ROW16 = false>
__global__ __launch_bounds__(512) void maxsim_pairs_kernel(const float* __restrict__ D, int dim, const float* __restrict__ Q, int nq,
                                                            int64_t q_stride, const int64_t* __restrict__ offsets,
                                                            const int32_t* __restrict__ candidates, int64_t n_items, int64_t item_stride,
                                                            float* __restrict__ out) {
    extern __shared__ __attribute__((aligned(16))) float qs[];
// ... 31 lines not shown
            for (int j = 0; j < NL; ++j) x[j] = (FULL || t0 + 16 * j < dim) ? *reinterpret_cast<const f32x4*>(a + 16 * j) : (f32x4){0.f, 0.f, 0.f, 0.f};
        }
    };
    auto lane_i64 = [](int64_t v, int k) __attribute__((always_inline)) {
        const uint32_t lo = __builtin_amdgcn_readlane((uint32_t)(uint64_t)v, k), hi = __builtin_amdgcn_readlane((uint32_t)((uint64_t)v >> 32), k);
        return (int64_t)(((uint64_t)hi << 32) | lo);
    };
    f32x4 xc[NL], xn[NL];
    for (int64_t base = (int64_t)blockIdx.x * 8 + w; base < n_items; base += 64 * stride) {
        const int64_t mine = base + (int64_t)lane * stride;
        int64_t vb = 0, ve = 0;
        if (mine < n_items) {
            const int64_t chunk = cb[mine];
            if (chunk >= 0) { vb = offsets[chunk]; ve = offsets[chunk + 1]; }
            if (ve <= vb) ob[mine] = -INFINITY;
        }
        const uint64_t todo = __builtin_amdgcn_ballot_w64(ve > vb);
        if (todo == 0ull) continue;
        int k = __builtin_ctzll(todo);
        int64_t e = lane_i64(ve, k), r0 = lane_i64(vb, k);
        int t0 = 0;
        request(xc, e, r0, 0);
        f32x4 y0 = *reinterpret_cast<const f32x4*>(q0), y1 = *reinterpret_cast<const f32x4*>(q1);
        float best0 = -INFINITY, best1 = -INFINITY;
        f32x4 acc0 = (f32x4){0.f, 0.f, 0.f, 0.f}, acc1 = acc0;
        for (;;) {
            const bool more_k = t0 + KB < dim, more_rows = r0 + 16 < e;
            const uint64_t rest = todo & ~((2ull << k) - 1ull);
            const int nk = rest ? __builtin_ctzll(rest) : k;
            const int64_t ne = lane_i64(ve, nk), nb = lane_i64(vb, nk);
            const int64_t n_e = (more_k || more_rows) ? e : ne;
            const int64_t n_r0 = more_k ? r0 : (more_rows ? r0 + 16 : nb);
            const int n_t0 = more_k ? t0 + KB : 0;
            request(xn, n_e, n_r0, n_t0);
            __builtin_amdgcn_sched_barrier(0);
#pragma unroll
            for (int j = 0; j < NL; ++j) {
                if (!FULL && t0 + 16 * j >= dim) break;
                const int tn = j + 1 < NL ? t0 + 16 * (j + 1) : n_t0;
                const int tr = (FULL || tn < dim) ? tn : 0;
                const f32x4 z0 = *reinterpret_cast<const f32x4*>(q0 + tr);
                const f32x4 z1 = *reinterpret_cast<const f32x4*>(q1 + tr);
                __builtin_amdgcn_sched_barrier(0);
#pragma unroll
                for (int u = 0; u < 4; ++u) {
                    acc0 = __builtin_amdgcn_mfma_f32_16x16x4f32(xc[j][u], y0[u], acc0, 0, 0, 0);
                    acc1 = __builtin_amdgcn_mfma_f32_16x16x4f32(xc[j][u], y1[u], acc1, 0, 0, 0);
                }
                __builtin_amdgcn_sched_barrier(0);
                y0 = z0;
                y1 = z1;
            }
            bool last = false;
            if (!more_k) {
                float v0 = -INFINITY, v1 = -INFINITY;
#pragma unroll
                for (int i = 0; i < 4; ++i)
                    if (r0 + 4 * g + i < e) { v0 = fmaxf(v0, acc0[i]); v1 = fmaxf(v1, acc1[i]); }
                v0 = fmaxf(v0, __shfl_xor(v0, 16)); v0 = fmaxf(v0, __shfl_xor(v0, 32));
                v1 = fmaxf(v1, __shfl_xor(v1, 16)); v1 = fmaxf(v1, __shfl_xor(v1, 32));
                best0 = fmaxf(best0, v0);
                best1 = fmaxf(best1, v1);
                acc0 = acc1 = (f32x4){0.f, 0.f, 0.f, 0.f};
                if (!more_rows) {
                    float s0 = best0, s1 = best1;
#pragma unroll
                    for (int o = 1; o < 16; o <<= 1) { s0 += __shfl_xor(s0, o); s1 += __shfl_xor(s1, o); }
                    if (lane == 0) ob[base + (int64_t)k * stride] = s0 + s1;
                    best0 = best1 = -INFINITY;
                    last = rest == 0ull;
                    k = nk;
                }
            }
            if (last) break;
            e = n_e;
            r0 = n_r0;
            t0 = n_t0;
#pragma unroll
            for (int j = 0; j < NL; ++j) xc[j] = xn[j];
        }
    }
}

template <int KB, bool ROW16, int DBG = 0, int NW = 8>
__global__ __launch_bounds__(NW * 64) void maxsim_pairs_packed_kernel(const float* __restrict__ D, int dim, const float* __restrict__ Q, int nq,
                                                                   int64_t q_stride, const int64_t* __restrict__ offsets,
                                                                   const int32_t* __restrict__ candidates, int64_t n_items, int64_t item_stride,
                                                                   float* __restrict__ out) {
    extern __shared__ __attribute__((aligned(16))) float qs[];
    const int pitch = dim + 8;
    const float* Qb = Q + (int64_t)blockIdx.y * q_stride;
    const int32_t* cb = candidates + (int64_t)blockIdx.y * item_stride;
    float* ob = out + (int64_t)blockIdx.y * item_stride;
    if constexpr ((DBG & 16) != 0) return;
    for (int i = threadIdx.x * 4; i < 32 * dim && !(DBG & 4); i += NW * 64 * 4) {
        const int n = i / dim, c = i - n * dim;
        f32x4 v = (f32x4){0.f, 0.f, 0.f, 0.f};
        if (n < nq) v = *reinterpret_cast<const f32x4*>(Qb + (int64_t)n * dim + c);
        *reinterpret_cast<f32x4*>(qs + n * pitch + c) = v;
    }
    __syncthreads();
    if constexpr ((DBG & 8) != 0) return;
    const int lane = threadIdx.x & 63, w = wave_id();
    const int m = lane & 15, g = lane >> 4;
    const float* q0 = qs + m * pitch + 4 * g;
    const float* q1 = qs + (16 + m) * pitch + 4 * g;
    const int64_t stride = (int64_t)gridDim.x * NW;
    constexpr int NL = KB / 16;
    auto request = [&](f32x4 (&x)[NL], int32_t row, int t0) __attribute__((always_inline)) {
        if constexpr ((DBG & 2) != 0) row = m;
        if constexpr (ROW16) {
            typedef _Float16 h16x4 __attribute__((ext_vector_type(4)));
            const _Float16* a = reinterpret_cast<const _Float16*>(D) + (int64_t)row * dim + 4 * g + t0;
#pragma unroll
            for (int j = 0; j < NL; ++j) {
                const h16x4 h = *reinterpret_cast<const h16x4*>(a + 16 * j);
                x[j] = (f32x4){(float)h[0], (float)h[1], (float)h[2], (float)h[3]};
            }
        } else {
            const float* a = D + (int64_t)row * dim + 4 * g + t0;
#pragma unroll
            for (int j = 0; j < NL; ++j) x[j] = *reinterpret_cast<const f32x4*>(a + 16 * j);
        }
    };
    f32x4 xc[NL], xn[NL];
    for (int64_t base = (int64_t)blockIdx.x * NW + w; base < n_items; base += 64 * stride) {
        const int64_t mine = base + (int64_t)lane * stride;
        int32_t vb = 0, ve = 0;
        if (mine < n_items) {
            const int64_t chunk = cb[mine];
            if (chunk >= 0) { vb = (int32_t)offsets[chunk]; ve = (int32_t)offsets[chunk + 1]; }
            if (ve <= vb) ob[mine] = -INFINITY;
        }
        const uint64_t todo = __builtin_amdgcn_ballot_w64(ve > vb);
        if (todo == 0ull) continue;
        uint32_t t_lo = ve > vb ? (uint32_t)(ve - vb) & 0xffffu : 0u, t_hi = ve > vb ? (uint32_t)(ve - vb) >> 16 : 0u;
#pragma unroll
        for (int o = 32; o > 0; o >>= 1) { t_lo += __shfl_xor(t_lo, o); t_hi += __shfl_xor(t_hi, o); }
        const int64_t R = ((int64_t)__builtin_amdgcn_readfirstlane(t_hi) << 16) + (int64_t)__builtin_amdgcn_readfirstlane(t_lo);
        const int64_t n_tiles = (R + 15) >> 4;
        int cur = __builtin_ctzll(todo);
        uint64_t rest = todo & (todo - 1ull);
        int32_t cur_row = __builtin_amdgcn_readlane(vb, cur), cur_end = __builtin_amdgcn_readlane(ve, cur);
        auto next_tile = [&](int32_t& row, int& cand) __attribute__((always_inline)) -> uint32_t {
            uint32_t ends = 0u;
            row = cur_row;
            cand = cur;
#pragma unroll
            for (int sl = 0; sl < 16; ++sl) {
                if (cur >= 0) {
                    if (m == sl) { row = cur_row; cand = cur; }
                    if (++cur_row == cur_end) {
                        ends |= 1u << sl;
                        if (rest != 0ull) {
                            cur = __builtin_ctzll(rest);
                            rest &= rest - 1ull;
                            cur_row = __builtin_amdgcn_readlane(vb, cur);
                            cur_end = __builtin_amdgcn_readlane(ve, cur);
                        } else {
                            cur = -1;
                        }
                    }
                }
            }
            return ends;
        };
        int32_t row_c, row_n = 0;
        int cand_c, cand_n = 0;
        uint32_t ends_c = next_tile(row_c, cand_c), ends_n = 0u;
        int64_t tile = 0;
        int t0 = 0;
        request(xc, row_c, 0);
        f32x4 y0 = *reinterpret_cast<const f32x4*>(q0), y1 = *reinterpret_cast<const f32x4*>(q1);
        float carry0 = -INFINITY, carry1 = -INFINITY;
        f32x4 acc0 = (f32x4){0.f, 0.f, 0.f, 0.f}, acc1 = acc0;
        for (;;) {
            const bool more_k = t0 + KB < dim, more_tiles = tile + 1 < n_tiles;
            if (!more_k && more_tiles) ends_n = next_tile(row_n, cand_n);
            const int32_t n_row = (more_k || !more_tiles) ? row_c : row_n;
            const int n_t0 = more_k ? t0 + KB : 0;
            request(xn, n_row, n_t0);
            __builtin_amdgcn_sched_barrier(0);
#pragma unroll
            for (int j = 0; j < NL; ++j) {
                const int tn = j + 1 < NL ? t0 + 16 * (j + 1) : n_t0;
                const f32x4 z0 = *reinterpret_cast<const f32x4*>(q0 + tn);
                const f32x4 z1 = *reinterpret_cast<const f32x4*>(q1 + tn);
                __builtin_amdgcn_sched_barrier(0);
                if constexpr ((DBG & 1) != 0) {
                    acc0 += xc[j] * y0;
                    acc1 += xc[j] * y1;
                } else {
#pragma unroll
                    for (int u = 0; u < 4; ++u) {
                        acc0 = __builtin_amdgcn_mfma_f32_16x16x4f32(xc[j][u], y0[u], acc0, 0, 0, 0);
                        acc1 = __builtin_amdgcn_mfma_f32_16x16x4f32(xc[j][u], y1[u], acc1, 0, 0, 0);
                    }
                }
                __builtin_amdgcn_sched_barrier(0);
                y0 = z0;
                y1 = z1;
            }
            if (!more_k) {
                const int n_valid = R - 16 * tile < 16 ? (int)(R - 16 * tile) : 16;
                uint32_t em = ends_c;
                int s_lo = 0;
                while (s_lo < n_valid) {
                    const bool closes = em != 0u;
                    const int e = closes ? __builtin_ctz(em) : 15;
                    float v0 = -INFINITY, v1 = -INFINITY;
#pragma unroll
                    for (int i = 0; i < 4; ++i)
                        if (4 * g + i >= s_lo && 4 * g + i <= e) { v0 = fmaxf(v0, acc0[i]); v1 = fmaxf(v1, acc1[i]); }
                    v0 = fmaxf(v0, __shfl_xor(v0, 16)); v0 = fmaxf(v0, __shfl_xor(v0, 32));
                    v1 = fmaxf(v1, __shfl_xor(v1, 16)); v1 = fmaxf(v1, __shfl_xor(v1, 32));
                    const float best0 = fmaxf(carry0, v0), best1 = fmaxf(carry1, v1);
                    if (closes) {
                        float s0 = best0, s1 = best1;
#pragma unroll
                        for (int o = 1; o < 16; o <<= 1) { s0 += __shfl_xor(s0, o); s1 += __shfl_xor(s1, o); }
                        const int c = __builtin_amdgcn_readlane(cand_c, e);
                        if (lane == 0) ob[base + (int64_t)c * stride] = s0 + s1;
                        carry0 = carry1 = -INFINITY;
                        em &= em - 1u;
                    } else {
                        carry0 = best0;
                        carry1 = best1;
                    }
                    s_lo = e + 1;
                }
                acc0 = acc1 = (f32x4){0.f, 0.f, 0.f, 0.f};
                if (!more_tiles) break;
                ++tile;
                row_c = row_n;
                cand_c = cand_n;
                ends_c = ends_n;
            }
            t0 = n_t0;
#pragma unroll
            for (int j = 0; j < NL; ++j) xc[j] = xn[j];
        }
    }
}

constexpr int PW_KW = 128, PW_T = 8, PW_PITCH = PW_KW + 8;
template <bool ROW16>
__global__ __launch_bounds__(512) void maxsim_pairs_wide_kernel(const float* __restrict__ D, int dim, const float* __restrict__ Q, int nq,
                                                                 int64_t q_stride, const int64_t* __restrict__ offsets,
                                                                 const int32_t* __restrict__ candidates, int64_t n_items, int64_t item_stride,
                                                                 float* __restrict__ out, const uint32_t* __restrict__ run_if) {
    extern __shared__ __attribute__((aligned(16))) float qs[];
    if (run_if && __builtin_amdgcn_readfirstlane((int)*run_if) == 0) return;
    const float* Qb = Q + (int64_t)blockIdx.y * q_stride;
    const int32_t* cb = candidates ? candidates + (int64_t)blockIdx.y * item_stride : nullptr;
    float* ob = out + (int64_t)blockIdx.y * item_stride;
    const int lane = threadIdx.x & 63, w = wave_id();
    const int m = lane & 15, g = lane >> 4;
    float* const qw = qs + w * 32 * PW_PITCH;
    const float* q0 = qw + m * PW_PITCH + 4 * g;
    const float* q1 = qw + (16 + m) * PW_PITCH + 4 * g;
    const int64_t stride = (int64_t)gridDim.x * 8;
    const int nwin = dim / PW_KW;
    constexpr int NL = PW_KW / 16;
    auto request = [&](f32x4 (&x)[NL], int32_t row, int t0) __attribute__((always_inline)) {
        if constexpr (ROW16) {
            typedef _Float16 h16x4 __attribute__((ext_vector_type(4)));
            const _Float16* a = reinterpret_cast<const _Float16*>(D) + (int64_t)row * dim + 4 * g + t0;
#pragma unroll
            for (int j = 0; j < NL; ++j) {
                const h16x4 h = *reinterpret_cast<const h16x4*>(a + 16 * j);
                x[j] = (f32x4){(float)h[0], (float)h[1], (float)h[2], (float)h[3]};
            }
        } else {
            const float* a = D + (int64_t)row * dim + 4 * g + t0;
#pragma unroll
            for (int j = 0; j < NL; ++j) x[j] = *reinterpret_cast<const f32x4*>(a + 16 * j);
        }
    };
    f32x4 xc[NL], xn[NL];
    for (int64_t base = (int64_t)blockIdx.x * 8 + w; base < n_items; base += 64 * stride) {
        const int64_t mine = base + (int64_t)lane * stride;
        int32_t vb = 0, ve = 0;
        if (mine < n_items) {
            const int64_t chunk = cb ? (int64_t)cb[mine] : mine;
            if (chunk >= 0) { vb = (int32_t)offsets[chunk]; ve = (int32_t)offsets[chunk + 1]; }
            if (ve <= vb) ob[mine] = -INFINITY;
        }
        const uint64_t todo = __builtin_amdgcn_ballot_w64(ve > vb);
        if (todo == 0ull) continue;
        uint32_t t_lo = ve > vb ? (uint32_t)(ve - vb) & 0xffffu : 0u, t_hi = ve > vb ? (uint32_t)(ve - vb) >> 16 : 0u;
#pragma unroll
        for (int o = 32; o > 0; o >>= 1) { t_lo += __shfl_xor(t_lo, o); t_hi += __shfl_xor(t_hi, o); }
        const int64_t R = ((int64_t)__builtin_amdgcn_readfirstlane(t_hi) << 16) + (int64_t)__builtin_amdgcn_readfirstlane(t_lo);
        const int64_t n_tiles = (R + 15) >> 4;
        int cur = __builtin_ctzll(todo);
        uint64_t rest = todo & (todo - 1ull);
        int32_t cur_row = __builtin_amdgcn_readlane(vb, cur), cur_end = __builtin_amdgcn_readlane(ve, cur);
        auto next_tile = [&](int32_t& row, int& cand) __attribute__((always_inline)) -> uint32_t {
            uint32_t ends = 0u;
            row = cur_row;
            cand = cur;
#pragma unroll
            for (int sl = 0; sl < 16; ++sl) {
                if (cur >= 0) {
                    if (m == sl) { row = cur_row; cand = cur; }
                    if (++cur_row == cur_end) {
                        ends |= 1u << sl;
                        if (rest != 0ull) {
                            cur = __builtin_ctzll(rest);
                            rest &= rest - 1ull;
                            cur_row = __builtin_amdgcn_readlane(vb, cur);
                            cur_end = __builtin_amdgcn_readlane(ve, cur);
                        } else {
                            cur = -1;
                        }
                    }
                }
            }
            return ends;
        };
        float carry0 = -INFINITY, carry1 = -INFINITY;
        for (int64_t tile0 = 0; tile0 < n_tiles; tile0 += PW_T) {
            const int gt = (int)(n_tiles - tile0 < PW_T ? n_tiles - tile0 : PW_T);
            int32_t row[PW_T];
// ... 6 lines not shown
            }
            f32x4 acc[PW_T][2];
#pragma unroll
            for (int t = 0; t < PW_T; ++t) acc[t][0] = acc[t][1] = (f32x4){0.f, 0.f, 0.f, 0.f};
            request(xc, row[0], 0);
            for (int kw = 0; kw < nwin; ++kw) {
                __builtin_amdgcn_wave_barrier();
#pragma unroll
                for (int j = 0; j < 16; ++j) {
                    const int i = j * 64 + lane, n = i >> 5, c = (i & 31) * 4;
                    f32x4 v = (f32x4){0.f, 0.f, 0.f, 0.f};
                    if (n < nq) v = *reinterpret_cast<const f32x4*>(Qb + (int64_t)n * dim + kw * PW_KW + c);
                    *reinterpret_cast<f32x4*>(qw + n * PW_PITCH + c) = v;
                }
                __builtin_amdgcn_wave_barrier();
#pragma unroll
                for (int t = 0; t < PW_T; ++t) {
                    if (t < gt) {
                        const bool last_t = t + 1 >= gt;
                        const int32_t n_row = (t + 1 < PW_T && !last_t) ? row[t + 1 < PW_T ? t + 1 : 0] : row[0];
                        const int n_t0 = last_t ? (kw + 1 < nwin ? (kw + 1) * PW_KW : 0) : kw * PW_KW;
                        request(xn, n_row, n_t0);
                        f32x4 y0 = *reinterpret_cast<const f32x4*>(q0), y1 = *reinterpret_cast<const f32x4*>(q1);
                        __builtin_amdgcn_sched_barrier(0);
#pragma unroll
                        for (int j = 0; j < NL; ++j) {
                            const int tn = j + 1 < NL ? 16 * (j + 1) : 0;
                            const f32x4 z0 = *reinterpret_cast<const f32x4*>(q0 + tn);
                            const f32x4 z1 = *reinterpret_cast<const f32x4*>(q1 + tn);
                            __builtin_amdgcn_sched_barrier(0);
#pragma unroll
                            for (int u = 0; u < 4; ++u) {
                                acc[t][0] = __builtin_amdgcn_mfma_f32_16x16x4f32(xc[j][u], y0[u], acc[t][0], 0, 0, 0);
                                acc[t][1] = __builtin_amdgcn_mfma_f32_16x16x4f32(xc[j][u], y1[u], acc[t][1], 0, 0, 0);
                            }
                            __builtin_amdgcn_sched_barrier(0);
                            y0 = z0;
                            y1 = z1;
                        }
#pragma unroll
                        for (int j = 0; j < NL; ++j) xc[j] = xn[j];
                    }
                }
            }
#pragma unroll
            for (int t = 0; t < PW_T; ++t) {
                if (t < gt) {
                    const int64_t tile = tile0 + t;
                    const int n_valid = R - 16 * tile < 16 ? (int)(R - 16 * tile) : 16;
                    uint32_t em = ends[t];
                    int s_lo = 0;
                    while (s_lo < n_valid) {
                        const bool closes = em != 0u;
                        const int e = closes ? __builtin_ctz(em) : 15;
                        float v0 = -INFINITY, v1 = -INFINITY;
#pragma unroll
                        for (int i = 0; i < 4; ++i)
                            if (4 * g + i >= s_lo && 4 * g + i <= e) { v0 = fmaxf(v0, acc[t][0][i]); v1 = fmaxf(v1, acc[t][1][i]); }
                        v0 = fmaxf(v0, __shfl_xor(v0, 16)); v0 = fmaxf(v0, __shfl_xor(v0, 32));
                        v1 = fmaxf(v1, __shfl_xor(v1, 16)); v1 = fmaxf(v1, __shfl_xor(v1, 32));
                        const float best0 = fmaxf(carry0, v0), best1 = fmaxf(carry1, v1);
                        if (closes) {
                            float s0 = best0, s1 = best1;
#pragma unroll
                            for (int o = 1; o < 16; o <<= 1) { s0 += __shfl_xor(s0, o); s1 += __shfl_xor(s1, o); }
                            const int c = __builtin_amdgcn_readlane(cand[t], e);
                            if (lane == 0) ob[base + (int64_t)c * stride] = s0 + s1;
                            carry0 = carry1 = -INFINITY;
                            em &= em - 1u;
                        } else {
                            carry0 = best0;
                            carry1 = best1;
                        }
                        s_lo = e + 1;
                    }
                }
            }
        }
    }
}

int launch_maxsim_pairs(const float* D, int32_t dim, const float* Q, int32_t nq, int64_t q_stride, const int64_t* offsets,
                        const int32_t* candidates, int64_t n_items_per_query, int32_t n_queries, float* out, hipStream_t s, bool rows16,
                        int64_t item_stride, int64_t first_item, int packed_mode) {
    bool packed = packed_mode != 0;
    if (n_items_per_query <= 0 || n_queries <= 0) return RL_OK;
    if (item_stride <= 0) item_stride = n_items_per_query;
    if (first_item < 0 || first_item + n_items_per_query > item_stride) return RL_ERR_INVALID;
    if (candidates) candidates += first_item;
    if (out) out += first_item;
    if (nq < 1 || nq > 32 || dim % 16 || dim < 16 || dim > PAIRS_MAX_DIM || !candidates) return RL_ERR_UNSUPPORTED;
    if ((reinterpret_cast<uintptr_t>(D) & (rows16 ? 7 : 15)) || (reinterpret_cast<uintptr_t>(Q) & 15) || (q_stride & 3)) return RL_ERR_UNSUPPORTED;
    if (dim > 1024) {
        if (dim % PW_KW) return RL_ERR_UNSUPPORTED;
        const size_t lds_w = (size_t)8 * 32 * PW_PITCH * sizeof(float);
        static bool wide_attr = false;
        if (!wide_attr) {
            RL_HIP(hipFuncSetAttribute(reinterpret_cast<const void*>(maxsim_pairs_wide_kernel<false>), hipFuncAttributeMaxDynamicSharedMemorySize, 160 * 1024));
            RL_HIP(hipFuncSetAttribute(reinterpret_cast<const void*>(maxsim_pairs_wide_kernel<true>), hipFuncAttributeMaxDynamicSharedMemorySize, 160 * 1024));
            wide_attr = true;
        }
        const int per_q = (int)std::max<int64_t>(1, std::min<int64_t>((n_items_per_query + 7) / 8, std::max<int64_t>(1, 256 / n_queries)));
        if (rows16)
            hipLaunchKernelGGL(maxsim_pairs_wide_kernel<true>, dim3(per_q, n_queries), dim3(512), lds_w, s, D, (int)dim, Q, (int)nq, q_stride, offsets,
                               candidates, n_items_per_query, item_stride, out, (const uint32_t*)nullptr);
        else
            hipLaunchKernelGGL(maxsim_pairs_wide_kernel<false>, dim3(per_q, n_queries), dim3(512), lds_w, s, D, (int)dim, Q, (int)nq, q_stride, offsets,
                               candidates, n_items_per_query, item_stride, out, (const uint32_t*)nullptr);
        RL_HIP(hipGetLastError());
        return RL_OK;
    }
    const size_t lds = (size_t)32 * (dim + 8) * sizeof(float);
    static bool attr_set = false;
    if (!attr_set) {
#define RL_PAIRS_ATTR(...) RL_HIP(hipFuncSetAttribute(reinterpret_cast<const void*>(maxsim_pairs_kernel<__VA_ARGS__>), hipFuncAttributeMaxDynamicSharedMemorySize, 160 * 1024))
#define RL_PACKED_ATTR(...) RL_HIP(hipFuncSetAttribute(reinterpret_cast<const void*>(maxsim_pairs_packed_kernel<__VA_ARGS__>), hipFuncAttributeMaxDynamicSharedMemorySize, 160 * 1024))
        RL_PACKED_ATTR(256, false);
        RL_PACKED_ATTR(128, false);
        RL_PACKED_ATTR(256, true);
        RL_PACKED_ATTR(128, true);
        RL_HIP(hipFuncSetAttribute(reinterpret_cast<const void*>(maxsim_pairs_packed_kernel<128, false, 0, 16>), hipFuncAttributeMaxDynamicSharedMemorySize, 160 * 1024));
#undef RL_PACKED_ATTR
        RL_PAIRS_ATTR(true, 256, false);
        RL_PAIRS_ATTR(true, 128, false);
        RL_PAIRS_ATTR(false, 128, false);
        RL_PAIRS_ATTR(true, 256, true);
        RL_PAIRS_ATTR(true, 128, true);
        RL_PAIRS_ATTR(false, 128, true);
#undef RL_PAIRS_ATTR
        attr_set = true;
    }
    const bool full = dim % 128 == 0;
    packed = packed && full;
    const bool wide = packed && packed_mode == 2 && !rows16;
    const int nw = wide ? 16 : 8;
    int per_query = (int)std::max<int64_t>(1, std::min<int64_t>((n_items_per_query + nw - 1) / nw, std::max<int64_t>(1, (packed ? 256 : 512) / n_queries)));
#ifdef RAGLITE_EXPERIMENTS
    if (const char* e = exp_env("RAGLITE_PAIRS_WG_BUDGET")) {
        const int budget = std::atoi(e);
        if (budget > 0) per_query = (int)std::max<int64_t>(1, std::min<int64_t>((n_items_per_query + 7) / 8, std::max<int64_t>(1, budget / n_queries)));
    }
#endif
#define RL_PAIRS(FULL_, KB_)                                                                                                               \
    do {                                                                                                                                   \
        if (rows16)                                                                                                                        \
            hipLaunchKernelGGL((maxsim_pairs_kernel<FULL_, KB_, true>), dim3(per_query, n_queries), dim3(512), lds, s, D, (int)dim, Q, (int)nq, \
                               q_stride, offsets, candidates, n_items_per_query, item_stride, out);                                        \
        else                                                                                                                               \
            hipLaunchKernelGGL((maxsim_pairs_kernel<FULL_, KB_, false>), dim3(per_query, n_queries), dim3(512), lds, s, D, (int)dim, Q, (int)nq, \
                               q_stride, offsets, candidates, n_items_per_query, item_stride, out);                                        \
    } while (0)
#define RL_PACKED(KB_)                                                                                                                     \
    do {                                                                                                                                   \
        if (rows16)                                                                                                                        \
            hipLaunchKernelGGL((maxsim_pairs_packed_kernel<KB_, true>), dim3(per_query, n_queries), dim3(512), lds, s, D, (int)dim, Q, (int)nq, \
                               q_stride, offsets, candidates, n_items_per_query, item_stride, out);                                        \
        else                                                                                                                               \
            hipLaunchKernelGGL((maxsim_pairs_packed_kernel<KB_, false>), dim3(per_query, n_queries), dim3(512), lds, s, D, (int)dim, Q, (int)nq, \
                               q_stride, offsets, candidates, n_items_per_query, item_stride, out);                                        \
    } while (0)
#ifdef RAGLITE_EXPERIMENTS
    static const int pdbg = exp_env("RAGLITE_PAIRS_DBG") ? std::atoi(exp_env("RAGLITE_PAIRS_DBG")) : 0;
    if (packed && dim % 256 == 0 && !rows16 && pdbg) {
#define RL_PDBG(D_) hipLaunchKernelGGL((maxsim_pairs_packed_kernel<256, false, D_>), dim3(per_query, n_queries), dim3(512), lds, s, D, (int)dim, Q, (int)nq, \
                                       q_stride, offsets, candidates, n_items_per_query, item_stride, out)
        static bool dbg_attr = false;
        if (!dbg_attr) {
            RL_HIP(hipFuncSetAttribute(reinterpret_cast<const void*>(maxsim_pairs_packed_kernel<256, false, 1>), hipFuncAttributeMaxDynamicSharedMemorySize, 160 * 1024));
            RL_HIP(hipFuncSetAttribute(reinterpret_cast<const void*>(maxsim_pairs_packed_kernel<256, false, 2>), hipFuncAttributeMaxDynamicSharedMemorySize, 160 * 1024));
            RL_HIP(hipFuncSetAttribute(reinterpret_cast<const void*>(maxsim_pairs_packed_kernel<256, false, 3>), hipFuncAttributeMaxDynamicSharedMemorySize, 160 * 1024));
            RL_HIP(hipFuncSetAttribute(reinterpret_cast<const void*>(maxsim_pairs_packed_kernel<256, false, 4>), hipFuncAttributeMaxDynamicSharedMemorySize, 160 * 1024));
            RL_HIP(hipFuncSetAttribute(reinterpret_cast<const void*>(maxsim_pairs_packed_kernel<256, false, 7>), hipFuncAttributeMaxDynamicSharedMemorySize, 160 * 1024));
            RL_HIP(hipFuncSetAttribute(reinterpret_cast<const void*>(maxsim_pairs_packed_kernel<256, false, 8>), hipFuncAttributeMaxDynamicSharedMemorySize, 160 * 1024));
            RL_HIP(hipFuncSetAttribute(reinterpret_cast<const void*>(maxsim_pairs_packed_kernel<256, false, 16>), hipFuncAttributeMaxDynamicSharedMemorySize, 160 * 1024));
            dbg_attr = true;
        }
        if (pdbg == 1) RL_PDBG(1); else if (pdbg == 2) RL_PDBG(2); else if (pdbg == 3) RL_PDBG(3); else if (pdbg == 4) RL_PDBG(4); else if (pdbg == 8) RL_PDBG(8);
        else if (pdbg == 16) RL_PDBG(16); else RL_PDBG(7);
#undef RL_PDBG
        RL_HIP(hipGetLastError());
        return RL_OK;
    }
#endif
    if (wide)
        hipLaunchKernelGGL((maxsim_pairs_packed_kernel<128, false, 0, 16>), dim3(per_query, n_queries), dim3(1024), lds, s, D, (int)dim, Q, (int)nq, q_stride,
                           offsets, candidates, n_items_per_query, item_stride, out);
    else if (packed && dim % 256 == 0) RL_PACKED(256);
    else if (packed && dim % 128 == 0) RL_PACKED(128);
    else if (dim % 256 == 0) RL_PAIRS(true, 256);
    else if (dim % 128 == 0) RL_PAIRS(true, 128);
    else RL_PAIRS(false, 128);
#undef RL_PACKED
#undef RL_PAIRS
    RL_HIP(hipGetLastError());
    return RL_OK;
}

int launch_maxsim_pairs_all_wide(const float* D, int32_t dim, const float* Q, int32_t nq, int64_t q_stride, const int64_t* offsets, int64_t n_chunks,
                                 int32_t n_queries, float* out, int64_t out_stride, hipStream_t s, const uint32_t* run_if, bool rows16) {
    if (n_chunks <= 0 || n_queries <= 0) return RL_OK;
    if (nq < 1 || nq > 32 || dim <= 1024 || dim > PAIRS_MAX_DIM || dim % PW_KW) return RL_ERR_UNSUPPORTED;
    if ((reinterpret_cast<uintptr_t>(D) & (rows16 ? 7 : 15)) || (reinterpret_cast<uintptr_t>(Q) & 15) || (q_stride & 3)) return RL_ERR_UNSUPPORTED;
    static bool attr = false;
    if (!attr) {
        RL_HIP(hipFuncSetAttribute(reinterpret_cast<const void*>(maxsim_pairs_wide_kernel<false>), hipFuncAttributeMaxDynamicSharedMemorySize, 160 * 1024));
        RL_HIP(hipFuncSetAttribute(reinterpret_cast<const void*>(maxsim_pairs_wide_kernel<true>), hipFuncAttributeMaxDynamicSharedMemorySize, 160 * 1024));
        attr = true;
    }
    const size_t lds_w = (size_t)8 * 32 * PW_PITCH * sizeof(float);
    const int per_q = (int)std::max<int64_t>(1, std::min<int64_t>((n_chunks + 511) / 512, std::max<int64_t>(1, 1024 / n_queries)));
    if (rows16)
        hipLaunchKernelGGL(maxsim_pairs_wide_kernel<true>, dim3(per_q, n_queries), dim3(512), lds_w, s, D, (int)dim, Q, (int)nq, q_stride, offsets,
                           (const int32_t*)nullptr, n_chunks, out_stride, out, run_if);
    else
    hipLaunchKernelGGL(maxsim_pairs_wide_kernel<false>, dim3(per_q, n_queries), dim3(512), lds_w, s, D, (int)dim, Q, (int)nq, q_stride, offsets,
                       (const int32_t*)nullptr, n_chunks, out_stride, out, run_if);
    RL_HIP(hipGetLastError());
    return RL_OK;
}

int launch_maxsim_generic(const float* D, int32_t dim, const float* Q, int32_t nq, int64_t q_stride,
                          const int64_t* offsets, const int32_t* candidates, int64_t n_items_per_query,
                          int32_t n_queries, float* out, hipStream_t s) {
    if (nq < 1 || nq > GEN_NQ_MAX) return fail(RL_ERR_UNSUPPORTED, "MaxSim: nq must be in [1, 1024]");
    if (n_items_per_query <= 0 || n_queries <= 0) return RL_OK;
    const bool vec4 = (dim % 4 == 0) && ((reinterpret_cast<uintptr_t>(D) & 15) == 0) &&
                      ((reinterpret_cast<uintptr_t>(Q) & 15) == 0) && ((q_stride * 4) % 16 == 0);
    for (int32_t qi = 0; qi < n_queries; ++qi) {
        const float* Qq = Q + (int64_t)qi * q_stride;
        const int32_t* cq = candidates ? candidates + (int64_t)qi * n_items_per_query : nullptr;
        float* oq = out + (int64_t)qi * n_items_per_query;
        int st = RL_ERR_UNSUPPORTED;
        if (vec4) {
            const int nv = (dim + 255) / 256;
            if (nv <= 1) st = generic_t<1, 4>(D, dim, Qq, nq, offsets, cq, n_items_per_query, oq, s);
            else if (nv <= 2) st = generic_t<2, 4>(D, dim, Qq, nq, offsets, cq, n_items_per_query, oq, s);
            else if (nv <= 4) st = generic_t<4, 4>(D, dim, Qq, nq, offsets, cq, n_items_per_query, oq, s);
            else if (nv <= 8) st = generic_t<8, 4>(D, dim, Qq, nq, offsets, cq, n_items_per_query, oq, s);
            else if (nv <= 16) st = generic_t<16, 4>(D, dim, Qq, nq, offsets, cq, n_items_per_query, oq, s);
        } else {
            const int nv = (dim + 63) / 64;
            if (nv <= 2) st = generic_t<2, 1>(D, dim, Qq, nq, offsets, cq, n_items_per_query, oq, s);
            else if (nv <= 8) st = generic_t<8, 1>(D, dim, Qq, nq, offsets, cq, n_items_per_query, oq, s);
            else if (nv <= 32) st = generic_t<32, 1>(D, dim, Qq, nq, offsets, cq, n_items_per_query, oq, s);
        }
        if (st == RL_ERR_UNSUPPORTED) return fail(RL_ERR_UNSUPPORTED, "MaxSim: dim too large for the generic kernel");
        RL_TRY(st);
    }
    return RL_OK;
}

constexpr int CD = 128;
constexpr int CPW = 8;

template <int NQT, bool F16, bool SPLIT = false>
__global__ __launch_bounds__(256) void maxsim_cand_kernel(const float* __restrict__ D, const float* __restrict__ Q,
                                                           int nq, const int64_t* __restrict__ offsets,
                                                           const int32_t* __restrict__ candidates, int n_cand,
                                                           int n_queries, float* __restrict__ out, float e_scale) {
    static_assert(!(F16 && SPLIT), "SPLIT is a way to multiply an fp32-stored corpus");
    const int lane = threadIdx.x & 63;
    const int fj = lane & 15, kq = lane >> 4;
    const int groups = (n_cand + CPW - 1) / CPW;
    const int64_t wave = (int64_t)blockIdx.x * 4 + (threadIdx.x >> 6);
    if (wave >= (int64_t)n_queries * groups) return;
    const int qi = (int)(wave / groups);
    const int c0 = (int)(wave % groups) * CPW;

    constexpr bool H = F16 || SPLIT;
// ... 109 lines not shown
                    for (int h = 0; h < NQT; ++h) acl[h] = __builtin_amdgcn_mfma_f32_16x16x32_f16(el, qhi[h][m], acl[h], 0, 0, 0);
                    if (any_lo) {
#pragma unroll
                        for (int h = 0; h < NQT; ++h) acl[h] = __builtin_amdgcn_mfma_f32_16x16x32_f16(eh, qlo[h][m], acl[h], 0, 0, 0);
                    }
                }
#pragma unroll
                for (int h = 0; h < NQT; ++h) acc[h] = (acc[h] + acl[h]) * q_unscale;
            } else if constexpr (!F16) {
                const float* p = D + row * CD + 4 * kq;
                f32x4 a[8];
#pragma unroll
                for (int mm = 0; mm < 8; ++mm) a[mm] = *reinterpret_cast<const f32x4*>(p + 16 * mm);
#pragma unroll
                for (int mm = 0; mm < 8; ++mm)
#pragma unroll
                    for (int tt = 0; tt < 4; ++tt)
#pragma unroll
                        for (int h = 0; h < NQT; ++h)
                            acc[h] = __builtin_amdgcn_mfma_f32_16x16x4f32(a[mm][tt], qreg[h][4 * mm + tt], acc[h], 0, 0, 0);
            } else {
                const uint16_t* p = reinterpret_cast<const uint16_t*>(D) + row * CD + 8 * kq;
                h16x8 a[4];
#pragma unroll
                for (int mm = 0; mm < 4; ++mm) a[mm] = *reinterpret_cast<const h16x8*>(p + 32 * mm);
#pragma unroll
                for (int mm = 0; mm < 4; ++mm)
#pragma unroll
                    for (int h = 0; h < NQT; ++h)
                        acc[h] = __builtin_amdgcn_mfma_f32_16x16x32_f16(a[mm], qhi[h][mm], acc[h], 0, 0, 0);
                if (any_lo) {
#pragma unroll
                    for (int mm = 0; mm < 4; ++mm)
#pragma unroll
                        for (int h = 0; h < NQT; ++h)
                            acc[h] = __builtin_amdgcn_mfma_f32_16x16x32_f16(a[mm], qlo[h][mm], acc[h], 0, 0, 0);
                }
            }
#pragma unroll
            for (int h = 0; h < NQT; ++h)
#pragma unroll
                for (int r = 0; r < 4; ++r) {
                    const bool valid = (r0 + 4 * kq + r) < e;
                    mx[h][r] = fmaxf(mx[h][r], valid ? acc[h][r] : -INFINITY);
                }
        }
        float s = 0.f;
#pragma unroll
        for (int h = 0; h < NQT; ++h) {
            float v = fmaxf(fmaxf(mx[h][0], mx[h][1]), fmaxf(mx[h][2], mx[h][3]));
            v = fmaxf(v, __shfl_xor(v, 16, 64));
            v = fmaxf(v, __shfl_xor(v, 32, 64));
            s += (16 * h + fj < nq) ? v : 0.f;
        }
        s += __shfl_xor(s, 1, 64);
        s += __shfl_xor(s, 2, 64);
        s += __shfl_xor(s, 4, 64);
        s += __shfl_xor(s, 8, 64);
        if (lane == 0) out[(int64_t)qi * n_cand + ci] = (e > b) ? s : -INFINITY;
    }
}

static int launch_cand_any(const float* D, bool f16, int32_t dim, const float* Q, int32_t nq, const int64_t* offsets,
                           const int32_t* candidates, int32_t n_cand, int32_t n_queries, float* out, hipStream_t s,
                           float split_scale = 0.f) {
    if (dim != CD || nq < 1 || nq > 32) return RL_ERR_UNSUPPORTED;
    if ((reinterpret_cast<uintptr_t>(D) & 15) || (reinterpret_cast<uintptr_t>(Q) & 15)) return RL_ERR_UNSUPPORTED;
    if (n_cand <= 0 || n_queries <= 0) return RL_OK;
    const int64_t waves = (int64_t)n_queries * ((n_cand + CPW - 1) / CPW);
    const int64_t blocks = (waves + 3) / 4;
    if (blocks > 0x7fffffff) return fail(RL_ERR_UNSUPPORTED, "MaxSim rerank: too many (query, candidate) pairs per launch");
#define RL_CAND(NQT, ...) hipLaunchKernelGGL((maxsim_cand_kernel<NQT, __VA_ARGS__>), dim3((unsigned)blocks), dim3(256), 0, s, D, Q, \
                                             (int)nq, offsets, candidates, (int)n_cand, (int)n_queries, out, split_scale)
    if (f16) { if (nq <= 16) RL_CAND(1, true); else RL_CAND(2, true); }
    else if (split_scale > 0.f) { if (nq <= 16) RL_CAND(1, false, true); else RL_CAND(2, false, true); }
    else     { if (nq <= 16) RL_CAND(1, false); else RL_CAND(2, false); }
#undef RL_CAND
    RL_HIP(hipGetLastError());
    return RL_OK;
}

__global__ __launch_bounds__(256) void sanitize_candidates_kernel(const int32_t* __restrict__ in, int64_t n, int64_t n_chunks,
                                                                   const uint32_t* __restrict__ live_chunk_bits,
                                                                   int32_t* __restrict__ out) {
    const int64_t i = (int64_t)blockIdx.x * blockDim.x + threadIdx.x;
    if (i >= n) return;
    const int32_t c = in[i];
    bool ok = c >= 0 && c < n_chunks;
    if (ok && live_chunk_bits) ok = (live_chunk_bits[c >> 5] >> (c & 31)) & 1u;
    out[i] = ok ? c : -1;
}
int launch_sanitize_candidates(const int32_t* in, int64_t n, int64_t n_chunks, const uint32_t* live_chunk_bits, int32_t* out,
                               hipStream_t s) {
    if (n <= 0) return RL_OK;
    hipLaunchKernelGGL(sanitize_candidates_kernel, dim3((unsigned)((n + 255) / 256)), dim3(256), 0, s, in, n, n_chunks, live_chunk_bits, out);
    RL_HIP(hipGetLastError());
    return RL_OK;
}

int launch_maxsim_cand(const float* D, int32_t dim, const float* Q, int32_t nq, const int64_t* offsets,
                       const int32_t* candidates, int32_t n_cand, int32_t n_queries, float* out, hipStream_t s,
                       float split_scale) {
    return launch_cand_any(D, false, dim, Q, nq, offsets, candidates, n_cand, n_queries, out, s, split_scale);
}

int launch_maxsim_cand16(const uint16_t* D, int32_t dim, const float* Q, int32_t nq, const int64_t* offsets,
                         const int32_t* candidates, int32_t n_cand, int32_t n_queries, float* out, hipStream_t s) {
    return launch_cand_any(reinterpret_cast<const float*>(D), true, dim, Q, nq, offsets, candidates, n_cand, n_queries,
                           out, s);
}

}
```

Before: 18260.

## Flatten MaxSim pair rerank into count-aware load-balanced persistent workgroups

```diff
diff --git a/include/raglite_hip.h b/include/raglite_hip.h
--- a/include/raglite_hip.h
+++ b/include/raglite_hip.h
@@ -83,7 +83,7 @@
     RL_OPT_F16_EXACT = 21, RL_OPT_LAZY_IMAGES = 22, RL_OPT_FUSED_PP_SAMPLE = 23,
     RL_OPT_LIST_SELECT = 24, RL_OPT_HI_FEW = 25, RL_OPT_TOPK_BLOCK = 26, RL_OPT_HI_PIVOT = 27, RL_OPT_COUNT_ = 28
 } rl_option;
-enum { RL_OPT_PP_SCHEDULE = 64, RL_OPT_PP_XCD_PASSES = 65 };
+enum { RL_OPT_PP_SCHEDULE = 64, RL_OPT_PP_XCD_PASSES = 65, RL_OPT_PAIRS_FLAT = 66 };
 int rl_set_default_option(int key, int64_t value);
 int rl_get_default_option(int key, int64_t* value);
 int rl_index_set_option(rl_index* index, int key, int64_t value);
@@ -122,6 +122,8 @@
 
 int rl_maxsim_rerank(rl_index* index, const float* query_vecs, int32_t n_queries, int32_t nq,
                      const int32_t* candidates, int32_t n_cand, float* out_scores, int mem, void* stream);
+int rl_maxsim_rerank_counted(rl_index* index, const float* query_vecs, int32_t n_queries, int32_t nq, const int32_t* candidates, int32_t n_cand,
+                             const uint32_t* counts, int32_t n_workgroups, float* out_scores, int mem, void* stream);
 
 int rl_merge_topk(const float* in_scores, const int32_t* in_ids, int32_t n_lists, int32_t n_queries,
                   int32_t k_in, int32_t k, float* out_scores, int32_t* out_ids, int mem, void* stream);
diff --git a/raglite_amd/_abi.py b/raglite_amd/_abi.py
--- a/raglite_amd/_abi.py
+++ b/raglite_amd/_abi.py
@@ -19,7 +19,7 @@
     "image_headroom_mb": 15, "arithmetic": 16, "exact_kth_threshold": 17, "fused_two_rounds": 18,
     "keep_hi_plane": 19, "pairs_packed": 20, "f16_exact": 21, "lazy_images": 22, "fused_pp_sample": 23, "list_select": 24, "hi_few": 25, "topk_block": 26, "hi_pivot": 27,
 }
-SCHEDULE_OPTIONS = {"pp_schedule": 64, "pp_xcd_passes": 65}
+SCHEDULE_OPTIONS = {"pp_schedule": 64, "pp_xcd_passes": 65, "pairs_flat": 66}
 
 
 def option_key(name: str) -> int:
@@ -81,6 +81,7 @@
     "rl_maxsim_batch_begin": [c_void_p, c_void_p, c_i32, c_i32, c_i32, c_void_p, c_int, c_void_p],
     "rl_maxsim_batch_finish": [c_void_p, c_void_p, c_void_p, c_i32, c_i32, c_void_p, c_void_p, c_int, c_void_p],
     "rl_maxsim_rerank": [c_void_p, c_void_p, c_i32, c_i32, c_void_p, c_i32, c_void_p, c_int, c_void_p],
+    "rl_maxsim_rerank_counted": [c_void_p, c_void_p, c_i32, c_i32, c_void_p, c_i32, c_void_p, c_i32, c_void_p, c_int, c_void_p],
     "rl_merge_topk": [c_void_p, c_void_p, c_i32, c_i32, c_i32, c_i32, c_void_p, c_void_p, c_int, c_void_p],
     "rl_topk": [c_void_p, c_i32, c_i64, c_i64, c_i32, c_void_p, c_void_p, c_int, c_void_p],
     "rl_time_kernel": [c_void_p, c_int, c_void_p, c_i32, c_i32, C.POINTER(C.c_float), c_void_p],
diff --git a/raglite_amd/_ops.py b/raglite_amd/_ops.py
--- a/raglite_amd/_ops.py
+++ b/raglite_amd/_ops.py
@@ -967,6 +967,26 @@
         check(lib().rl_maxsim_rerank(self._handle, p_q, n_queries, nq, p_c, n_cand, p_s, a.mem, a.stream))
         return o_s
 
+    def maxsim_rerank_counted(self, query_vecs, candidates, counts, n_workgroups: int = 0):
+        a = _Args()
+        p_q = a.inp(query_vecs, np.float32)
+        qv = a.keep[-1]
+        if qv.ndim != 3 or int(qv.shape[2]) != self.dim:
+            raise ValueError("query_vecs must be (n_queries, nq, dim)")
+        p_c = a.inp(candidates, np.int32)
+        cv = a.keep[-1]
+        n_queries, nq = int(qv.shape[0]), int(qv.shape[1])
+        if cv.ndim != 2 or int(cv.shape[0]) != n_queries:
+            raise ValueError("candidates must be (n_queries, n_cand)")
+        p_n = a.inp(counts, np.int32)
+        if a.keep[-1].ndim != 1 or int(a.keep[-1].shape[0]) != n_queries:
+            raise ValueError("counts must be (n_queries,)")
+        n_cand = int(cv.shape[1])
+        o_s, p_s = a.out((n_queries, n_cand), np.float32)
+        self._prep(a)
+        check(lib().rl_maxsim_rerank_counted(self._handle, p_q, n_queries, nq, p_c, n_cand, p_n, int(n_workgroups), p_s, a.mem, a.stream))
+        return o_s
+
     def chunk_best_rows(self, queries, candidates):
         a = _Args()
         p_q, B, single = self._queries(a, queries)
diff --git a/raglite_amd/csrc/api.hip b/raglite_amd/csrc/api.hip
--- a/raglite_amd/csrc/api.hip
+++ b/raglite_amd/csrc/api.hip
@@ -206,7 +206,7 @@
 constexpr size_t SCORE_BATCH_BYTES = size_t(8) << 30;
 
 struct Options {
-    int64_t v[RL_OPT_PP_XCD_PASSES + 1];
+    int64_t v[RL_OPT_PAIRS_FLAT + 1];
     Options() {
         for (auto& x : v) x = 0;
         v[RL_OPT_HI_SEARCH] = v[RL_OPT_HI_MAXSIM] = v[RL_OPT_HI_PRODUCTS] = v[RL_OPT_PP_PASS] = v[RL_OPT_FUSED_TOPK] = v[RL_OPT_FUSED_HI] = 1;
@@ -216,6 +216,7 @@
         v[RL_OPT_HI_PIVOT] = 1;
         v[RL_OPT_PP_SCHEDULE] = 1;
         v[RL_OPT_PP_XCD_PASSES] = 2;
+        v[RL_OPT_PAIRS_FLAT] = 1;
         v[RL_OPT_IMAGE_HEADROOM_MB] = -1;
         v[RL_OPT_ARITHMETIC] = RL_ARITH_AUTO;
     }
@@ -223,13 +224,13 @@
 };
 std::mutex g_default_opts_mu;
 Options g_default_opts;
-bool option_key_ok(int key) { return (key >= 1 && key < RL_OPT_COUNT_) || key == RL_OPT_PP_SCHEDULE || key == RL_OPT_PP_XCD_PASSES; }
+bool option_key_ok(int key) { return (key >= 1 && key < RL_OPT_COUNT_) || key == RL_OPT_PP_SCHEDULE || key == RL_OPT_PP_XCD_PASSES || key == RL_OPT_PAIRS_FLAT; }
 bool option_value_ok(int key, int64_t value) {
     switch (key) {
         case RL_OPT_HI_SEARCH: case RL_OPT_HI_MAXSIM: case RL_OPT_PP_PASS: case RL_OPT_FUSED_TOPK: case RL_OPT_FUSED_HI: case RL_OPT_FUSED_PP:
         case RL_OPT_GEMM_PASS: case RL_OPT_QUERY_PAIRS: case RL_OPT_PLANES_GEMM: case RL_OPT_KEEP_IMAGE: case RL_OPT_KEEP_HI:
         case RL_OPT_EXACT_KTH_THRESHOLD: case RL_OPT_FUSED_TWO_ROUNDS: case RL_OPT_KEEP_HI_PLANE: case RL_OPT_F16_EXACT: case RL_OPT_LAZY_IMAGES: case RL_OPT_FUSED_PP_SAMPLE: case RL_OPT_LIST_SELECT: case RL_OPT_HI_FEW: case RL_OPT_HI_PIVOT:
-        case RL_OPT_PP_SCHEDULE:
+        case RL_OPT_PP_SCHEDULE: case RL_OPT_PAIRS_FLAT:
             return value == 0 || value == 1;
         case RL_OPT_PP_XCD_PASSES: return value == 8 || value == 4 || value == 2 || value == 1;
         case RL_OPT_TOPK_BLOCK: case RL_OPT_PAIRS_PACKED: return value >= 0 && value <= 2;
@@ -2047,10 +2048,11 @@
     const bool rows16 = idx->E16 != nullptr;
     idx->filt = {RL_FILTER_MAXSIM_BATCH, n_gemm, hb.cap, hb.cnt, hb.flag};
     const int packed = (int)idx->opt.v[RL_OPT_PAIRS_PACKED];
+    const int flat = idx->opt.on(RL_OPT_PAIRS_FLAT) ? idx->n_cu : 0;
     const bool m_from_qsum = !hb.m_ready && hb.qsum != nullptr;
     if (!hb.m_ready && !(hb.exact_kth && k <= hb.cap && hb.qsum)) return fail(RL_ERR_INVALID, "MaxSim batch: no bound for the candidate threshold");
     if (hb.exact_kth && k <= hb.cap) {
-        RL_TRY(launch_maxsim_pairs(rows, idx->dim, d_q, nq, (int64_t)q_elems, idx->offsets, hb.ti, k, n_gemm, hb.es_top, s, rows16, 0, 0, packed));
+        RL_TRY(launch_maxsim_pairs(rows, idx->dim, d_q, nq, (int64_t)q_elems, idx->offsets, hb.ti, k, n_gemm, hb.es_top, s, rows16, 0, 0, packed, nullptr, 0, flat));
         if (m_from_qsum)
             RL_TRY(launch_exact_threshold(hb.es_top, hb.ti, n_gemm, k, hb.m, hb.cap, hb.thr, hb.cnt, hb.ci, hb.es, hb.flag, s, hb.qsum, hb.m_abs,
                                           idx->norm_stats.max_row_norm + idx->norm_stats.max_lo_norm, hb.one_product, hb.ts));
@@ -2058,11 +2060,12 @@
             RL_TRY(launch_exact_threshold(hb.es_top, hb.ti, n_gemm, k, hb.m, hb.cap, hb.thr, hb.cnt, hb.ci, hb.es, hb.flag, s, nullptr, 0.f, 0.f, false, hb.ts));
         RL_TRY(launch_collect_above(sc, n_gemm, idx->n_chunks, ld, hb.thr, nullptr, hb.cap, hb.ci, nullptr, hb.cnt, hb.flag, s, hb.ts, hb.ti, k));
         if (hb.cap > k)
-            RL_TRY(launch_maxsim_pairs(rows, idx->dim, d_q, nq, (int64_t)q_elems, idx->offsets, hb.ci, hb.cap - k, n_gemm, hb.es, s, rows16, hb.cap, k, packed));
+            RL_TRY(launch_maxsim_pairs(rows, idx->dim, d_q, nq, (int64_t)q_elems, idx->offsets, hb.ci, hb.cap - k, n_gemm, hb.es, s, rows16, hb.cap, k, packed,
+                                       hb.cnt, k, flat));
     } else {
         RL_HIP(hipMemsetAsync(hb.ci, 0xff, (size_t)n_gemm * hb.cap * sizeof(int32_t), s));
         RL_TRY(launch_collect_above(sc, n_gemm, idx->n_chunks, ld, hb.thr, nullptr, hb.cap, hb.ci, nullptr, hb.cnt, hb.flag, s));
-        RL_TRY(launch_maxsim_pairs(rows, idx->dim, d_q, nq, (int64_t)q_elems, idx->offsets, hb.ci, hb.cap, n_gemm, hb.es, s, rows16, 0, 0, packed));
+        RL_TRY(launch_maxsim_pairs(rows, idx->dim, d_q, nq, (int64_t)q_elems, idx->offsets, hb.ci, hb.cap, n_gemm, hb.es, s, rows16, 0, 0, packed, hb.cnt, 0, flat));
     }
     RL_TRY(launch_merge_topk(hb.es, hb.ci, 1, n_gemm, hb.cap, k, d_s, d_c, s, hb.cnt));
     return hi_batch_fallback(idx, d_q, nq, n_queries, n_gemm, k, sc, ld, hb, d_s, d_c, s, rows_only);
@@ -2464,6 +2467,34 @@
     RL_TRY(stage_in(candidates, (size_t)n_queries * n_cand, mem, s, t_c, &d_c));
     RL_TRY(stage_out_begin(out_scores, (size_t)n_queries * n_cand, mem, t_o, &d_o));
     RL_TRY(maxsim_rerank_device(idx, d_q, n_queries, nq, d_c, n_cand, d_o, s));
+    RL_TRY(stage_out_end(out_scores, (size_t)n_queries * n_cand, mem, s, t_o));
+    return finish(mem, s);
+}
+
+int rl_maxsim_rerank_counted(rl_index* idx, const float* query_vecs, int32_t n_queries, int32_t nq, const int32_t* candidates, int32_t n_cand,
+                             const uint32_t* counts, int32_t n_workgroups, float* out_scores, int mem, void* stream) {
+    if (!idx) return fail(RL_ERR_INVALID, "rl_maxsim_rerank_counted: null index");
+    if (n_queries < 0 || n_cand < 0 || nq < 1 || n_workgroups < 0) return fail(RL_ERR_INVALID, "rl_maxsim_rerank_counted: bad sizes");
+    if (n_queries == 0 || n_cand == 0) return RL_OK;
+    if (!query_vecs || !candidates || !counts || !out_scores) return fail(RL_ERR_INVALID, "rl_maxsim_rerank_counted: null argument");
+    hipStream_t s = as_stream(stream);
+    std::lock_guard<std::mutex> lock(idx->mu);
+    RL_TRY(use_scratch(idx, s));
+    DevBuf t_q, t_c, t_n, t_o;
+    const float* d_q; const int32_t* d_c; const uint32_t* d_n; float* d_o;
+    RL_TRY(stage_in(query_vecs, (size_t)n_queries * nq * idx->dim, mem, s, t_q, &d_q));
+    RL_TRY(stage_in(candidates, (size_t)n_queries * n_cand, mem, s, t_c, &d_c));
+    RL_TRY(stage_in(counts, (size_t)n_queries, mem, s, t_n, &d_n));
+    RL_TRY(stage_out_begin(out_scores, (size_t)n_queries * n_cand, mem, t_o, &d_o));
+    const int64_t n_items = (int64_t)n_queries * n_cand;
+    RL_TRY(idx->cand.reserve((size_t)n_items * sizeof(int32_t)));
+    RL_TRY(launch_sanitize_candidates(d_c, n_items, idx->n_chunks, idx->live_chunk_bits, idx->cand.as<int32_t>(), s, d_n, n_cand));
+    const int flat = idx->opt.on(RL_OPT_PAIRS_FLAT) ? (n_workgroups > 0 ? n_workgroups : idx->n_cu) : 0;
+    const int st = launch_maxsim_pairs(idx->E16 ? reinterpret_cast<const float*>(idx->E16) : idx->E, idx->dim, d_q, nq, (int64_t)nq * idx->dim, idx->offsets,
+                                       idx->cand.as<int32_t>(), n_cand, n_queries, d_o, s, idx->E16 != nullptr, 0, 0, (int)idx->opt.v[RL_OPT_PAIRS_PACKED],
+                                       d_n, 0, flat);
+    if (st == RL_ERR_UNSUPPORTED) return fail(st, "rl_maxsim_rerank_counted: needs nq <= 32 and dim % 16 == 0 (dim % 128 == 0 beyond 1024)");
+    if (st != RL_OK) return st;
     RL_TRY(stage_out_end(out_scores, (size_t)n_queries * n_cand, mem, s, t_o));
     return finish(mem, s);
 }
diff --git a/raglite_amd/csrc/common.h b/raglite_amd/csrc/common.h
--- a/raglite_amd/csrc/common.h
+++ b/raglite_amd/csrc/common.h
@@ -411,14 +411,15 @@
                         const int32_t* candidates, int64_t n_items_per_query, int32_t n_queries, float* out, hipStream_t s,
                         bool rows16 = false,
                         int64_t item_stride = 0, int64_t first_item = 0,
-                        int packed = 1);
+                        int packed = 1,
+                        const uint32_t* counts = nullptr, int32_t count_sub = 0, int flat_workgroups = 0);
 int launch_maxsim_pairs_all_wide(const float* D, int32_t dim, const float* Q, int32_t nq, int64_t q_stride, const int64_t* offsets, int64_t n_chunks,
                                  int32_t n_queries, float* out, int64_t out_stride, hipStream_t s, const uint32_t* run_if, bool rows16 = false);
 int launch_maxsim_generic(const float* D, int32_t dim, const float* Q, int32_t nq, int64_t q_stride_queries,
                           const int64_t* chunk_offsets, const int32_t* candidates, int64_t n_items,
                           int32_t n_queries, float* out, hipStream_t s);
 int launch_sanitize_candidates(const int32_t* in, int64_t n, int64_t n_chunks, const uint32_t* live_chunk_bits, int32_t* out,
-                               hipStream_t s);
+                               hipStream_t s, const uint32_t* counts = nullptr, int32_t n_cand = 0);
 int launch_maxsim_cand(const float* D, int32_t dim, const float* Q, int32_t nq, const int64_t* chunk_offsets,
                        const int32_t* candidates, int32_t n_cand, int32_t n_queries, float* out, hipStream_t s,
                        float split_scale = 0.f);
diff --git a/raglite_amd/csrc/maxsim_generic.hip b/raglite_amd/csrc/maxsim_generic.hip
--- a/raglite_amd/csrc/maxsim_generic.hip
+++ b/raglite_amd/csrc/maxsim_generic.hip
@@ -1,4 +1,6 @@
 #include "common.h"
+
+#include <type_traits>
 
 namespace rl {
 
@@ -196,30 +198,19 @@
     }
 }
 
-template <int KB, bool ROW16, int DBG = 0, int NW = 8>
+template <int KB, bool ROW16, int DBG = 0, int NW = 8, bool FLAT = false>
 __global__ __launch_bounds__(NW * 64) void maxsim_pairs_packed_kernel(const float* __restrict__ D, int dim, const float* __restrict__ Q, int nq,
                                                                    int64_t q_stride, const int64_t* __restrict__ offsets,
                                                                    const int32_t* __restrict__ candidates, int64_t n_items, int64_t item_stride,
-                                                                   float* __restrict__ out) {
+                                                                   float* __restrict__ out, const uint32_t* __restrict__ counts, int count_sub,
+                                                                   int n_queries) {
     extern __shared__ __attribute__((aligned(16))) float qs[];
     const int pitch = dim + 8;
-    const float* Qb = Q + (int64_t)blockIdx.y * q_stride;
-    const int32_t* cb = candidates + (int64_t)blockIdx.y * item_stride;
-    float* ob = out + (int64_t)blockIdx.y * item_stride;
     if constexpr ((DBG & 16) != 0) return;
-    for (int i = threadIdx.x * 4; i < 32 * dim && !(DBG & 4); i += NW * 64 * 4) {
-        const int n = i / dim, c = i - n * dim;
-        f32x4 v = (f32x4){0.f, 0.f, 0.f, 0.f};
-        if (n < nq) v = *reinterpret_cast<const f32x4*>(Qb + (int64_t)n * dim + c);
-        *reinterpret_cast<f32x4*>(qs + n * pitch + c) = v;
-    }
-    __syncthreads();
-    if constexpr ((DBG & 8) != 0) return;
     const int lane = threadIdx.x & 63, w = wave_id();
     const int m = lane & 15, g = lane >> 4;
     const float* q0 = qs + m * pitch + 4 * g;
     const float* q1 = qs + (16 + m) * pitch + 4 * g;
-    const int64_t stride = (int64_t)gridDim.x * NW;
     constexpr int NL = KB / 16;
     auto request = [&](f32x4 (&x)[NL], int32_t row, int t0) __attribute__((always_inline)) {
         if constexpr ((DBG & 2) != 0) row = m;
@@ -237,123 +228,218 @@
             for (int j = 0; j < NL; ++j) x[j] = *reinterpret_cast<const f32x4*>(a + 16 * j);
         }
     };
+    auto length_of = [&](int qq) __attribute__((always_inline)) -> int {
+        if (counts == nullptr) return (int)n_items;
+        const int64_t c = (int64_t)counts[qq] - count_sub;
+        return (int)(c < 0 ? 0 : (c > n_items ? n_items : c));
+    };
+    int q = blockIdx.y, q_len = (int)n_items, seg_a = 0, left = 0;
+    if constexpr (FLAT) {
+        for (int qq = blockIdx.x; qq < n_queries; qq += gridDim.x) {
+            float* o = out + (int64_t)qq * item_stride;
+            for (int64_t j = (int64_t)length_of(qq) + threadIdx.x; j < n_items; j += NW * 64) o[j] = -INFINITY;
+        }
+        int total = 0;
+        for (int qb = 0; qb < n_queries; qb += 64) {
+            int c = qb + lane < n_queries ? length_of(qb + lane) : 0;
+#pragma unroll
+            for (int o = 32; o > 0; o >>= 1) c += __shfl_xor(c, o);
+            total += __builtin_amdgcn_readfirstlane(c);
+        }
+        const int lo = (int)((int64_t)blockIdx.x * total / gridDim.x);
+        left = (int)((int64_t)(blockIdx.x + 1) * total / gridDim.x) - lo;
+        if (left <= 0) return;
+        int before = 0;
+        q = -1;
+        for (int qb = 0; qb < n_queries && q < 0; qb += 64) {
+            const int c = qb + lane < n_queries ? length_of(qb + lane) : 0;
+            int incl = c;
+#pragma unroll
+            for (int o = 1; o < 64; o <<= 1) {
+                const int t = __shfl_up(incl, o);
+                if (lane >= o) incl += t;
+            }
+            const uint64_t holds = __builtin_amdgcn_ballot_w64(before + incl > lo);
+            if (holds != 0ull) {
+                const int l = __builtin_ctzll(holds);
+                q = qb + l;
+                q_len = __builtin_amdgcn_readlane(c, l);
+                seg_a = lo - (before + __builtin_amdgcn_readlane(incl, l) - q_len);
+            }
+            before += __builtin_amdgcn_readlane(incl, 63);
+        }
+        if (q < 0) return;
+    }
     f32x4 xc[NL], xn[NL];
-    for (int64_t base = (int64_t)blockIdx.x * NW + w; base < n_items; base += 64 * stride) {
-        const int64_t mine = base + (int64_t)lane * stride;
-        int32_t vb = 0, ve = 0;
-        if (mine < n_items) {
-            const int64_t chunk = cb[mine];
-            if (chunk >= 0) { vb = (int32_t)offsets[chunk]; ve = (int32_t)offsets[chunk + 1]; }
-            if (ve <= vb) ob[mine] = -INFINITY;
-        }
-        const uint64_t todo = __builtin_amdgcn_ballot_w64(ve > vb);
-        if (todo == 0ull) continue;
-        uint32_t t_lo = ve > vb ? (uint32_t)(ve - vb) & 0xffffu : 0u, t_hi = ve > vb ? (uint32_t)(ve - vb) >> 16 : 0u;
-#pragma unroll
-        for (int o = 32; o > 0; o >>= 1) { t_lo += __shfl_xor(t_lo, o); t_hi += __shfl_xor(t_hi, o); }
-        const int64_t R = ((int64_t)__builtin_amdgcn_readfirstlane(t_hi) << 16) + (int64_t)__builtin_amdgcn_readfirstlane(t_lo);
-        const int64_t n_tiles = (R + 15) >> 4;
-        int cur = __builtin_ctzll(todo);
-        uint64_t rest = todo & (todo - 1ull);
-        int32_t cur_row = __builtin_amdgcn_readlane(vb, cur), cur_end = __builtin_amdgcn_readlane(ve, cur);
-        auto next_tile = [&](int32_t& row, int& cand) __attribute__((always_inline)) -> uint32_t {
-            uint32_t ends = 0u;
-            row = cur_row;
-            cand = cur;
-#pragma unroll
-            for (int sl = 0; sl < 16; ++sl) {
-                if (cur >= 0) {
-                    if (m == sl) { row = cur_row; cand = cur; }
-                    if (++cur_row == cur_end) {
-                        ends |= 1u << sl;
-                        if (rest != 0ull) {
-                            cur = __builtin_ctzll(rest);
-                            rest &= rest - 1ull;
-                            cur_row = __builtin_amdgcn_readlane(vb, cur);
-                            cur_end = __builtin_amdgcn_readlane(ve, cur);
-                        } else {
-                            cur = -1;
+    int32_t vb = 0, ve = 0;
+    uint64_t todo = 0ull, rest = 0ull;
+    int64_t tiles_left = 0;
+    int last_valid = 0;
+    int cur = 0;
+    int32_t cur_row = 0, cur_end = 0;
+    auto next_tile = [&](int32_t& row, int& cand) __attribute__((always_inline)) -> uint32_t {
+        uint32_t ends = 0u;
+        row = cur_row;
+        cand = cur;
+#pragma unroll
+        for (int sl = 0; sl < 16; ++sl) {
+            if (cur >= 0) {
+                if (m == sl) { row = cur_row; cand = cur; }
+                if (++cur_row == cur_end) {
+                    ends |= 1u << sl;
+                    if (rest != 0ull) {
+                        cur = __builtin_ctzll(rest);
+                        rest &= rest - 1ull;
+                        cur_row = __builtin_amdgcn_readlane(vb, cur);
+                        cur_end = __builtin_amdgcn_readlane(ve, cur);
+                    } else {
+                        cur = -1;
+                    }
+                }
+            }
+        }
+        return ends;
+    };
+    int32_t row_c = 0, row_n = 0;
+    int cand_c = 0, cand_n = 0;
+    uint32_t ends_c = 0u, ends_n = 0u;
+    for (;;) {
+        typedef typename std::conditional<FLAT, int, int64_t>::type item_t;
+        const item_t a = FLAT ? (item_t)seg_a : 0;
+        const item_t b = FLAT ? (item_t)(q_len - seg_a < left ? q_len : seg_a + left) : (item_t)n_items;
+        const item_t stride = FLAT ? (item_t)NW : (item_t)((int64_t)gridDim.x * NW);
+        const float* Qb = Q + (int64_t)q * q_stride;
+        const int32_t* cb = candidates + (int64_t)q * item_stride;
+        float* ob = out + (int64_t)q * item_stride;
+        auto open_batch = [&](item_t base) __attribute__((always_inline)) {
+            const item_t mine = base + (item_t)lane * stride;
+            vb = 0;
+            ve = 0;
+            if (mine < b) {
+                const int64_t chunk = cb[mine];
+                if (chunk >= 0) { vb = (int32_t)offsets[chunk]; ve = (int32_t)offsets[chunk + 1]; }
+                if (ve <= vb) ob[mine] = -INFINITY;
+            }
+            todo = __builtin_amdgcn_ballot_w64(ve > vb);
+            if (todo == 0ull) return;
+            uint32_t t_lo = ve > vb ? (uint32_t)(ve - vb) & 0xffffu : 0u, t_hi = ve > vb ? (uint32_t)(ve - vb) >> 16 : 0u;
+#pragma unroll
+            for (int o = 32; o > 0; o >>= 1) { t_lo += __shfl_xor(t_lo, o); t_hi += __shfl_xor(t_hi, o); }
+            const int64_t R = ((int64_t)__builtin_amdgcn_readfirstlane(t_hi) << 16) + (int64_t)__builtin_amdgcn_readfirstlane(t_lo);
+            tiles_left = (R + 15) >> 4;
+            last_valid = (int)(R - ((tiles_left - 1) << 4));
+            cur = __builtin_ctzll(todo);
+            rest = todo & (todo - 1ull);
+            cur_row = __builtin_amdgcn_readlane(vb, cur);
+            cur_end = __builtin_amdgcn_readlane(ve, cur);
+            ends_c = next_tile(row_c, cand_c);
+            request(xc, row_c, 0);
+        };
+        item_t base = a + (FLAT ? (item_t)w : (item_t)((int64_t)blockIdx.x * NW + w));
+        bool opened = base < b;
+        if (opened) open_batch(base);
+        __builtin_amdgcn_sched_barrier(0);
+        if (FLAT) __syncthreads();
+        for (int i0 = threadIdx.x * 4; i0 < 32 * dim && !(DBG & 4); i0 += NW * 64 * 4 * 4) {
+            f32x4 v[4];
+#pragma unroll
+            for (int u = 0; u < 4; ++u) {
+                const int i = i0 + u * NW * 64 * 4, n = i / dim, c = i - n * dim;
+                v[u] = (f32x4){0.f, 0.f, 0.f, 0.f};
+                if (n < nq) v[u] = *reinterpret_cast<const f32x4*>(Qb + (int64_t)n * dim + c);
+            }
+#pragma unroll
+            for (int u = 0; u < 4; ++u) {
+                const int i = i0 + u * NW * 64 * 4, n = i / dim, c = i - n * dim;
+                if (i < 32 * dim) *reinterpret_cast<f32x4*>(qs + n * pitch + c) = v[u];
+            }
+        }
+        __syncthreads();
+        if constexpr ((DBG & 8) != 0) return;
+        for (; base < b; base += 64 * stride) {
+            if (!opened) open_batch(base);
+            opened = false;
+            if (todo == 0ull) continue;
+            int t0 = 0;
+            f32x4 y0 = *reinterpret_cast<const f32x4*>(q0), y1 = *reinterpret_cast<const f32x4*>(q1);
+            float carry0 = -INFINITY, carry1 = -INFINITY;
+            f32x4 acc0 = (f32x4){0.f, 0.f, 0.f, 0.f}, acc1 = acc0;
+            for (;;) {
+                const bool more_k = t0 + KB < dim, more_tiles = tiles_left > 1;
+                if (!more_k && more_tiles) ends_n = next_tile(row_n, cand_n);
+                const int32_t n_row = (more_k || !more_tiles) ? row_c : row_n;
+                const int n_t0 = more_k ? t0 + KB : 0;
+                request(xn, n_row, n_t0);
+                __builtin_amdgcn_sched_barrier(0);
+#pragma unroll
+                for (int j = 0; j < NL; ++j) {
+                    const int tn = j + 1 < NL ? t0 + 16 * (j + 1) : n_t0;
+                    const f32x4 z0 = *reinterpret_cast<const f32x4*>(q0 + tn);
+                    const f32x4 z1 = *reinterpret_cast<const f32x4*>(q1 + tn);
+                    __builtin_amdgcn_sched_barrier(0);
+                    if constexpr ((DBG & 1) != 0) {
+                        acc0 += xc[j] * y0;
+                        acc1 += xc[j] * y1;
+                    } else {
+#pragma unroll
+                        for (int u = 0; u < 4; ++u) {
+                            acc0 = __builtin_amdgcn_mfma_f32_16x16x4f32(xc[j][u], y0[u], acc0, 0, 0, 0);
+                            acc1 = __builtin_amdgcn_mfma_f32_16x16x4f32(xc[j][u], y1[u], acc1, 0, 0, 0);
                         }
                     }
-                }
-            }
-            return ends;
-        };
-        int32_t row_c, row_n = 0;
-        int cand_c, cand_n = 0;
-        uint32_t ends_c = next_tile(row_c, cand_c), ends_n = 0u;
-        int64_t tile = 0;
-        int t0 = 0;
-        request(xc, row_c, 0);
-        f32x4 y0 = *reinterpret_cast<const f32x4*>(q0), y1 = *reinterpret_cast<const f32x4*>(q1);
-        float carry0 = -INFINITY, carry1 = -INFINITY;
-        f32x4 acc0 = (f32x4){0.f, 0.f, 0.f, 0.f}, acc1 = acc0;
-        for (;;) {
-            const bool more_k = t0 + KB < dim, more_tiles = tile + 1 < n_tiles;
-            if (!more_k && more_tiles) ends_n = next_tile(row_n, cand_n);
-            const int32_t n_row = (more_k || !more_tiles) ? row_c : row_n;
-            const int n_t0 = more_k ? t0 + KB : 0;
-            request(xn, n_row, n_t0);
-            __builtin_amdgcn_sched_barrier(0);
-#pragma unroll
-            for (int j = 0; j < NL; ++j) {
-                const int tn = j + 1 < NL ? t0 + 16 * (j + 1) : n_t0;
-                const f32x4 z0 = *reinterpret_cast<const f32x4*>(q0 + tn);
-                const f32x4 z1 = *reinterpret_cast<const f32x4*>(q1 + tn);
-                __builtin_amdgcn_sched_barrier(0);
-                if constexpr ((DBG & 1) != 0) {
-                    acc0 += xc[j] * y0;
-                    acc1 += xc[j] * y1;
-                } else {
-#pragma unroll
-                    for (int u = 0; u < 4; ++u) {
-                        acc0 = __builtin_amdgcn_mfma_f32_16x16x4f32(xc[j][u], y0[u], acc0, 0, 0, 0);
-                        acc1 = __builtin_amdgcn_mfma_f32_16x16x4f32(xc[j][u], y1[u], acc1, 0, 0, 0);
+                    __builtin_amdgcn_sched_barrier(0);
+                    y0 = z0;
+                    y1 = z1;
+                }
+                if (!more_k) {
+                    const int n_valid = more_tiles ? 16 : last_valid;
+                    uint32_t em = ends_c;
+                    int s_lo = 0;
+                    while (s_lo < n_valid) {
+                        const bool closes = em != 0u;
+                        const int e = closes ? __builtin_ctz(em) : 15;
+                        float v0 = -INFINITY, v1 = -INFINITY;
+#pragma unroll
+                        for (int i = 0; i < 4; ++i)
+                            if (4 * g + i >= s_lo && 4 * g + i <= e) { v0 = fmaxf(v0, acc0[i]); v1 = fmaxf(v1, acc1[i]); }
+                        v0 = fmaxf(v0, __shfl_xor(v0, 16)); v0 = fmaxf(v0, __shfl_xor(v0, 32));
+                        v1 = fmaxf(v1, __shfl_xor(v1, 16)); v1 = fmaxf(v1, __shfl_xor(v1, 32));
+                        const float best0 = fmaxf(carry0, v0), best1 = fmaxf(carry1, v1);
+                        if (closes) {
+                            float s0 = best0, s1 = best1;
+#pragma unroll
+                            for (int o = 1; o < 16; o <<= 1) { s0 += __shfl_xor(s0, o); s1 += __shfl_xor(s1, o); }
+                            const int c = __builtin_amdgcn_readlane(cand_c, e);
+                            if (lane == 0) ob[base + (item_t)c * stride] = s0 + s1;
+                            carry0 = carry1 = -INFINITY;
+                            em &= em - 1u;
+                        } else {
+                            carry0 = best0;
+                            carry1 = best1;
+                        }
+                        s_lo = e + 1;
                     }
-                }
-                __builtin_amdgcn_sched_barrier(0);
-                y0 = z0;
-                y1 = z1;
-            }
-            if (!more_k) {
-                const int n_valid = R - 16 * tile < 16 ? (int)(R - 16 * tile) : 16;
-                uint32_t em = ends_c;
-                int s_lo = 0;
-                while (s_lo < n_valid) {
-                    const bool closes = em != 0u;
-                    const int e = closes ? __builtin_ctz(em) : 15;
-                    float v0 = -INFINITY, v1 = -INFINITY;
-#pragma unroll
-                    for (int i = 0; i < 4; ++i)
-                        if (4 * g + i >= s_lo && 4 * g + i <= e) { v0 = fmaxf(v0, acc0[i]); v1 = fmaxf(v1, acc1[i]); }
-                    v0 = fmaxf(v0, __shfl_xor(v0, 16)); v0 = fmaxf(v0, __shfl_xor(v0, 32));
-                    v1 = fmaxf(v1, __shfl_xor(v1, 16)); v1 = fmaxf(v1, __shfl_xor(v1, 32));
-                    const float best0 = fmaxf(carry0, v0), best1 = fmaxf(carry1, v1);
-                    if (closes) {
-                        float s0 = best0, s1 = best1;
-#pragma unroll
-                        for (int o = 1; o < 16; o <<= 1) { s0 += __shfl_xor(s0, o); s1 += __shfl_xor(s1, o); }
-                        const int c = __builtin_amdgcn_readlane(cand_c, e);
-                        if (lane == 0) ob[base + (int64_t)c * stride] = s0 + s1;
-                        carry0 = carry1 = -INFINITY;
-                        em &= em - 1u;
-                    } else {
-                        carry0 = best0;
-                        carry1 = best1;
-                    }
-                    s_lo = e + 1;
-                }
-                acc0 = acc1 = (f32x4){0.f, 0.f, 0.f, 0.f};
-                if (!more_tiles) break;
-                ++tile;
-                row_c = row_n;
-                cand_c = cand_n;
-                ends_c = ends_n;
-            }
-            t0 = n_t0;
-#pragma unroll
-            for (int j = 0; j < NL; ++j) xc[j] = xn[j];
-        }
+                    acc0 = acc1 = (f32x4){0.f, 0.f, 0.f, 0.f};
+                    if (!more_tiles) break;
+                    --tiles_left;
+                    row_c = row_n;
+                    cand_c = cand_n;
+                    ends_c = ends_n;
+                }
+                t0 = n_t0;
+#pragma unroll
+                for (int j = 0; j < NL; ++j) xc[j] = xn[j];
+            }
+        }
+        if constexpr (!FLAT) break;
+        left -= (int)(b - a);
+        if (left <= 0) break;
+        seg_a = 0;
+        do {
+            ++q;
+            q_len = q < n_queries ? length_of(q) : 0;
+        } while (q < n_queries && q_len == 0);
+        if (q >= n_queries) break;
     }
 }
 
@@ -526,7 +612,7 @@
 
 int launch_maxsim_pairs(const float* D, int32_t dim, const float* Q, int32_t nq, int64_t q_stride, const int64_t* offsets,
                         const int32_t* candidates, int64_t n_items_per_query, int32_t n_queries, float* out, hipStream_t s, bool rows16,
-                        int64_t item_stride, int64_t first_item, int packed_mode) {
+                        int64_t item_stride, int64_t first_item, int packed_mode, const uint32_t* counts, int32_t count_sub, int flat_workgroups) {
     bool packed = packed_mode != 0;
     if (n_items_per_query <= 0 || n_queries <= 0) return RL_OK;
     if (item_stride <= 0) item_stride = n_items_per_query;
@@ -564,6 +650,7 @@
         RL_PACKED_ATTR(256, true);
         RL_PACKED_ATTR(128, true);
         RL_HIP(hipFuncSetAttribute(reinterpret_cast<const void*>(maxsim_pairs_packed_kernel<128, false, 0, 16>), hipFuncAttributeMaxDynamicSharedMemorySize, 160 * 1024));
+        RL_HIP(hipFuncSetAttribute(reinterpret_cast<const void*>(maxsim_pairs_packed_kernel<128, false, 0, 16, true>), hipFuncAttributeMaxDynamicSharedMemorySize, 160 * 1024));
 #undef RL_PACKED_ATTR
         RL_PAIRS_ATTR(true, 256, false);
         RL_PAIRS_ATTR(true, 128, false);
@@ -578,6 +665,8 @@
     packed = packed && full;
     const bool wide = packed && packed_mode == 2 && !rows16;
     const int nw = wide ? 16 : 8;
+    const bool flat = wide && flat_workgroups > 0 && (int64_t)n_queries * n_items_per_query < (int64_t(1) << 31);
+    const int flat_grid = std::min(flat_workgroups, 65535);
     int per_query = (int)std::max<int64_t>(1, std::min<int64_t>((n_items_per_query + nw - 1) / nw, std::max<int64_t>(1, (packed ? 256 : 512) / n_queries)));
 #ifdef RAGLITE_EXPERIMENTS
     if (const char* e = exp_env("RAGLITE_PAIRS_WG_BUDGET")) {
@@ -598,16 +687,32 @@
     do {                                                                                                                                   \
         if (rows16)                                                                                                                        \
             hipLaunchKernelGGL((maxsim_pairs_packed_kernel<KB_, true>), dim3(per_query, n_queries), dim3(512), lds, s, D, (int)dim, Q, (int)nq, \
-                               q_stride, offsets, candidates, n_items_per_query, item_stride, out);                                        \
+                               q_stride, offsets, candidates, n_items_per_query, item_stride, out, (const uint32_t*)nullptr, 0, (int)n_queries); \
         else                                                                                                                               \
             hipLaunchKernelGGL((maxsim_pairs_packed_kernel<KB_, false>), dim3(per_query, n_queries), dim3(512), lds, s, D, (int)dim, Q, (int)nq, \
-                               q_stride, offsets, candidates, n_items_per_query, item_stride, out);                                        \
+                               q_stride, offsets, candidates, n_items_per_query, item_stride, out, (const uint32_t*)nullptr, 0, (int)n_queries); \
     } while (0)
 #ifdef RAGLITE_EXPERIMENTS
     static const int pdbg = exp_env("RAGLITE_PAIRS_DBG") ? std::atoi(exp_env("RAGLITE_PAIRS_DBG")) : 0;
+    if (flat && (pdbg == 1 || pdbg == 2)) {
+        static bool flat_dbg_attr = false;
+        if (!flat_dbg_attr) {
+            RL_HIP(hipFuncSetAttribute(reinterpret_cast<const void*>(maxsim_pairs_packed_kernel<128, false, 1, 16, true>), hipFuncAttributeMaxDynamicSharedMemorySize, 160 * 1024));
+            RL_HIP(hipFuncSetAttribute(reinterpret_cast<const void*>(maxsim_pairs_packed_kernel<128, false, 2, 16, true>), hipFuncAttributeMaxDynamicSharedMemorySize, 160 * 1024));
+            flat_dbg_attr = true;
+        }
+        if (pdbg == 1)
+            hipLaunchKernelGGL((maxsim_pairs_packed_kernel<128, false, 1, 16, true>), dim3(flat_grid), dim3(1024), lds, s, D, (int)dim, Q, (int)nq, q_stride,
+                               offsets, candidates, n_items_per_query, item_stride, out, counts, (int)count_sub, (int)n_queries);
+        else
+            hipLaunchKernelGGL((maxsim_pairs_packed_kernel<128, false, 2, 16, true>), dim3(flat_grid), dim3(1024), lds, s, D, (int)dim, Q, (int)nq, q_stride,
+                               offsets, candidates, n_items_per_query, item_stride, out, counts, (int)count_sub, (int)n_queries);
+        RL_HIP(hipGetLastError());
+        return RL_OK;
+    }
     if (packed && dim % 256 == 0 && !rows16 && pdbg) {
 #define RL_PDBG(D_) hipLaunchKernelGGL((maxsim_pairs_packed_kernel<256, false, D_>), dim3(per_query, n_queries), dim3(512), lds, s, D, (int)dim, Q, (int)nq, \
-                                       q_stride, offsets, candidates, n_items_per_query, item_stride, out)
+                                       q_stride, offsets, candidates, n_items_per_query, item_stride, out, (const uint32_t*)nullptr, 0, (int)n_queries)
         static bool dbg_attr = false;
         if (!dbg_attr) {
             RL_HIP(hipFuncSetAttribute(reinterpret_cast<const void*>(maxsim_pairs_packed_kernel<256, false, 1>), hipFuncAttributeMaxDynamicSharedMemorySize, 160 * 1024));
@@ -626,9 +731,12 @@
         return RL_OK;
     }
 #endif
-    if (wide)
+    if (flat)
+        hipLaunchKernelGGL((maxsim_pairs_packed_kernel<128, false, 0, 16, true>), dim3(flat_grid), dim3(1024), lds, s, D, (int)dim, Q, (int)nq, q_stride,
+                           offsets, candidates, n_items_per_query, item_stride, out, counts, (int)count_sub, (int)n_queries);
+    else if (wide)
         hipLaunchKernelGGL((maxsim_pairs_packed_kernel<128, false, 0, 16>), dim3(per_query, n_queries), dim3(1024), lds, s, D, (int)dim, Q, (int)nq, q_stride,
-                           offsets, candidates, n_items_per_query, item_stride, out);
+                           offsets, candidates, n_items_per_query, item_stride, out, (const uint32_t*)nullptr, 0, (int)n_queries);
     else if (packed && dim % 256 == 0) RL_PACKED(256);
     else if (packed && dim % 128 == 0) RL_PACKED(128);
     else if (dim % 256 == 0) RL_PAIRS(true, 256);
@@ -904,18 +1012,20 @@
 
 __global__ __launch_bounds__(256) void sanitize_candidates_kernel(const int32_t* __restrict__ in, int64_t n, int64_t n_chunks,
                                                                    const uint32_t* __restrict__ live_chunk_bits,
-                                                                   int32_t* __restrict__ out) {
+                                                                   int32_t* __restrict__ out, const uint32_t* __restrict__ counts, int32_t n_cand) {
     const int64_t i = (int64_t)blockIdx.x * blockDim.x + threadIdx.x;
     if (i >= n) return;
     const int32_t c = in[i];
     bool ok = c >= 0 && c < n_chunks;
+    if (ok && counts) ok = (uint32_t)(i % n_cand) < counts[i / n_cand];
     if (ok && live_chunk_bits) ok = (live_chunk_bits[c >> 5] >> (c & 31)) & 1u;
     out[i] = ok ? c : -1;
 }
 int launch_sanitize_candidates(const int32_t* in, int64_t n, int64_t n_chunks, const uint32_t* live_chunk_bits, int32_t* out,
-                               hipStream_t s) {
+                               hipStream_t s, const uint32_t* counts, int32_t n_cand) {
     if (n <= 0) return RL_OK;
-    hipLaunchKernelGGL(sanitize_candidates_kernel, dim3((unsigned)((n + 255) / 256)), dim3(256), 0, s, in, n, n_chunks, live_chunk_bits, out);
+    if (counts && n_cand < 1) return RL_ERR_INVALID;
+    hipLaunchKernelGGL(sanitize_candidates_kernel, dim3((unsigned)((n + 255) / 256)), dim3(256), 0, s, in, n, n_chunks, live_chunk_bits, out, counts, n_cand);
     RL_HIP(hipGetLastError());
     return RL_OK;
 }
```

Result: no change. 18400 (median of 6 runs) (+0.8%).
